# gleb-kov/wordpiece

Measured on AMD Instinct MI355X. Metric: input MB/s tokenized (bert-base-cased vocab; offline stand-in: synthetic BERT-like vocab), higher is better.
Workload: dtype int32

## Files before the change

### include/wordpiece_amd.h

```cpp
#ifndef WORDPIECE_AMD_H
#define WORDPIECE_AMD_H

#include <stddef.h>
#include <stdint.h>

#ifdef __cplusplus
extern "C" {
#endif

#define WP_OK 0
#define WP_ERR_EMPTY_WORD 1
#define WP_ERR_TOO_LARGE 2
#define WP_ERR_HIP 3
#define WP_ERR_NO_DEVICE 4
#define WP_ERR_IO 5
#define WP_ERR_ARG 6

typedef struct wp_vocab wp_vocab;

int wp_vocab_create(const char *const *lines, const size_t *line_bytes, size_t n_lines,
                    wp_vocab **out);
int wp_vocab_create_packed(const char *buf, const int64_t *offsets, int64_t n_lines,
                           wp_vocab **out);
int wp_vocab_from_file(const char *vocab_file, wp_vocab **out);
// ... 33 lines not shown
typedef struct { int32_t max_len, cls_id, sep_id, pad_id, pairs, truncation, stride, unit; } wp_inputs_spec;
typedef struct { int32_t *input_ids, *token_type_ids, *lengths, *sample; uint32_t *offsets; } wp_inputs;
int wp_linear_encode_inputs(wp_vocab *v, const char *utf8, size_t nbytes, const int64_t *doc_off, size_t n_docs,
                            const wp_inputs_spec *spec, wp_inputs *out, size_t *n_out, size_t *n_samples);
int wp_linear_encode_inputs_device(wp_vocab *v, const void *d_utf8, size_t nbytes, const int64_t *d_doc_off, size_t n_docs,
                                   const wp_inputs_spec *spec, const wp_inputs *d_out, size_t capacity_rows,
                                   size_t *n_out, size_t *n_samples);

typedef struct { int32_t max_len, cls_id, sep_id, pad_id, mask_id, ignore_id, whole_word, reserved;
                 uint64_t select_q32, mask_q32, random_q32, seed, row_base; } wp_mask_spec;
int wp_word_ids(wp_vocab *v, const int32_t *input_ids, const int32_t *lengths, size_t n_rows, const wp_mask_spec *spec,
                int32_t **word_ids);
int wp_word_ids_device(wp_vocab *v, const int32_t *d_input_ids, const int32_t *d_lengths, size_t n_rows,
                       const wp_mask_spec *spec, int32_t *d_word_ids);
int wp_mlm_mask(wp_vocab *v, const int32_t *input_ids, const int32_t *lengths, size_t n_rows, const wp_mask_spec *spec,
                int32_t **masked, int32_t **labels, int32_t **word_ids);
int wp_mlm_mask_device(wp_vocab *v, const int32_t *d_input_ids, const int32_t *d_lengths, size_t n_rows,
                       const wp_mask_spec *spec, int32_t *d_masked, int32_t *d_labels, int32_t *d_word_ids);
typedef struct {
  int64_t n_rows;
  int64_t n_words;
  int64_t n_selected;
  int64_t n_selected_units;
  int64_t n_masked, n_random, n_kept;
  int32_t whole_word, reserved;
} wp_mask_stats;
int wp_get_mask_stats(const wp_vocab *v, wp_mask_stats *out);

typedef struct { int32_t max_len, cleanup, terminator, n_skip; int32_t skip_ids[8]; } wp_detok_spec;
int wp_detokenize(wp_vocab *v, const int32_t *ids, const int64_t *row_splits, const int32_t *lengths, size_t n_rows,
                  const wp_detok_spec *spec, char **text, int64_t **text_off, size_t *n_bytes);
int wp_detokenize_device(wp_vocab *v, const int32_t *d_ids, const int64_t *d_row_splits, const int32_t *d_lengths,
                         size_t n_rows, const wp_detok_spec *spec, const void **d_text, const int64_t **d_text_off,
                         size_t *n_bytes);
int64_t wp_detok_piece(const wp_vocab *v, int64_t id, int form, int cleanup, char *buf, size_t cap);
typedef struct { int64_t n_rows, n_cells, n_kept, n_skipped, n_dropped, n_bytes; } wp_detok_stats;
int wp_get_detok_stats(const wp_vocab *v, wp_detok_stats *out);

int wp_linear_encode_multi(wp_vocab *v, const char *utf8, size_t nbytes, const int *devices,
                           int n_devices, int32_t **ids, size_t *n_ids);

int wp_linear_encode_batch(wp_vocab *v, const char *const *texts, const size_t *nbytes, size_t n_texts,
                           int32_t **ids, size_t *n_ids);

typedef int (*wp_text_source)(void *user, size_t index, const char **utf8, size_t *nbytes);
typedef void (*wp_ids_sink)(void *user, size_t index, const int32_t *ids, size_t n_ids);
int wp_linear_encode_stream(wp_vocab *v, wp_text_source next, wp_ids_sink out, void *user);

int wp_reserve(wp_vocab *v, size_t nbytes);

int wp_trim(wp_vocab *v);

int wp_linear_encode_file(const char *text_file, const char *vocab_file, int32_t **ids,
                          size_t *n_ids);
int wp_linear_encode_external(const char *text_file, const char *vocab_file, const char *out_file,
                              size_t memory_limit);

int wp_fast_encode(wp_vocab *v, const char *utf8, size_t nbytes, int32_t **ids, size_t *n_ids);
int wp_fast_encode_device(wp_vocab *v, const void *d_utf8, size_t nbytes, const int32_t **d_ids,
                          size_t *n_ids);
int wp_fast_encode_file(const char *text_file, const char *vocab_file, int32_t **ids, size_t *n_ids);
int wp_fast_encode_external(const char *text_file, const char *vocab_file, const char *out_file,
                            size_t memory_limit);
int64_t wp_vocab_token_utf8(const wp_vocab *v, int64_t i, char *buf, size_t cap);

#define WP_OPT_FULL_DEPTH 1
#define WP_OPT_DEVICE 2
#define WP_OPT_KEEP_DEBUG 3
#define WP_OPT_STAGE_TIMING 4
#define WP_OPT_LCP_KASAI 5
#define WP_OPT_COVER_ANCHORS 7
#define WP_OPT_ARENA_GUARD 8
#define WP_OPT_DEVICES 9
#define WP_OPT_VOCAB_IN_S 10
#define WP_OPT_SPARSE_EMIT 11
#define WP_OPT_INDEXED_ROUND0 12
#define WP_OPT_SORT_BLANKS 13
#define WP_OPT_NORMALIZE 14
#define WP_NORM_CLEAN 1
#define WP_NORM_LOWER 2
#define WP_NORM_STRIP_ACCENTS 4
#define WP_NORM_BERT_UNCASED 7
#define WP_OPT_LATE_REFINE 15
int wp_set_option(wp_vocab *v, int option, int64_t value);

int wp_normalize_cp(int flags, uint32_t cp, uint32_t out[3]);
int wp_normalize_device(wp_vocab *v, const void *d_utf8, size_t nbytes, int flags, const void **d_out, size_t *out_bytes);
int wp_normalize(wp_vocab *v, const char *utf8, size_t nbytes, int flags, char **out, size_t *out_bytes);

typedef struct {
  int64_t n_bytes, n_text, n_total, alphabet, longest_token, n_ids;
  int32_t symbol_bits, symbols_per_key, rounds, sorted_depth, full_depth;
  int64_t radix_pass_elems;
  int32_t radix_passes;
  int64_t active_per_round[40];
  double ms_total, ms_decode, ms_sa, ms_lcp, ms_scan, ms_walk;
  double ms_radix_scatter;
  int64_t n_anchors;
  int32_t anchor_mode;
  double ms_h2d, ms_d2h;
  int64_t radix_digit_bytes;
  double ms_host_total;
  int32_t guard_zones;
  int32_t n_devices;
  int32_t vocab_in_s;
  int32_t reserved0;
  int64_t needed_after_round0;
  int32_t key_bits;
  int32_t staged_emit;
  int32_t rank_in_pass;
  int32_t trie_refine;
  int64_t arena_bytes;
  int32_t list_retries;
  int32_t hist_in_keys;
  int64_t radix_pass_bytes;
  int64_t round0_candidates;
  int32_t round0_keys_only;
  int32_t offsets_unit;
  int64_t round0_sorted;
  int64_t n_rows, rows_truncated;
  int32_t rows_route;
} wp_stats;
int wp_get_stats(const wp_vocab *v, wp_stats *out);
typedef struct {
  int32_t normalize;
  int64_t norm_bytes;
  double ms_normalize;
} wp_norm_stats;
int wp_get_norm_stats(const wp_vocab *v, wp_norm_stats *out);
typedef struct {
  int64_t n_wide_words;
  int64_t n_long_words;
  int32_t lean;
  int32_t max_anchor_gap;
} wp_walk_stats;
int wp_get_walk_stats(const wp_vocab *v, wp_walk_stats *out);
typedef struct {
  int64_t n_groups;
  int64_t n_entries;
  int64_t n_large_groups;
  int64_t n_large_entries;
  int64_t trie_nodes;
  int32_t sort_bits;
  int32_t key_lookup;
  int32_t symbol_bytes;
  int32_t reserved;
} wp_refine_stats;
int wp_get_refine_stats(const wp_vocab *v, wp_refine_stats *out);
typedef struct {
  int32_t early;
  int32_t reserved;
  double ms_sort_to_scan;
} wp_refine_sched;
int wp_get_refine_sched(const wp_vocab *v, wp_refine_sched *out);
typedef struct {
  int64_t n_samples, n_out;
  int64_t n_cut;
  int64_t n_windowed;
  int32_t pairs, truncation, stride, reserved;
} wp_inputs_stats;
int wp_get_inputs_stats(const wp_vocab *v, wp_inputs_stats *out);

int wp_linear_debug_fetch(const wp_vocab *v, int which, int32_t *out, size_t capacity,
                          size_t *n_out);

void wp_free(void *p);
const char *wp_last_error(void);
int wp_device_count(void);

#ifdef __cplusplus
}
#endif
#endif
```

### wordpiece_amd/__init__.py

```python
import ctypes as C
import os
import weakref

import numpy as np

_HERE = os.path.dirname(os.path.abspath(__file__))
LIB_PATH = os.environ.get("WP_LIB") or os.path.join(_HERE, "libwordpiece_amd.so")

WP_OPT_FULL_DEPTH, WP_OPT_DEVICE, WP_OPT_KEEP_DEBUG, WP_OPT_STAGE_TIMING, WP_OPT_LCP_KASAI = 1, 2, 3, 4, 5
WP_OPT_COVER_ANCHORS, WP_OPT_ARENA_GUARD, WP_OPT_DEVICES, WP_OPT_VOCAB_IN_S = 7, 8, 9, 10
WP_OPT_SPARSE_EMIT = 11
WP_OPT_INDEXED_ROUND0 = 12
WP_OPT_SORT_BLANKS = 13
WP_OPT_NORMALIZE = 14
WP_OPT_LATE_REFINE = 15
WP_NORM_CLEAN, WP_NORM_LOWER, WP_NORM_STRIP_ACCENTS, WP_NORM_BERT_UNCASED = 1, 2, 4, 7
WP_OFFSETS_BYTES, WP_OFFSETS_CODE_POINTS = 0, 1
_OFFSET_UNITS = {"byte": WP_OFFSETS_BYTES, "char": WP_OFFSETS_CODE_POINTS}
WP_TRUNC_LONGEST_FIRST, WP_TRUNC_ONLY_FIRST, WP_TRUNC_ONLY_SECOND = 0, 1, 2
_TRUNCATIONS = {"longest_first": WP_TRUNC_LONGEST_FIRST, "only_first": WP_TRUNC_ONLY_FIRST,
                "only_second": WP_TRUNC_ONLY_SECOND}

ABI_SYMBOLS = [
    "wp_vocab_create", "wp_vocab_create_packed", "wp_vocab_from_file", "wp_vocab_destroy", "wp_vocab_size",
    "wp_vocab_unk_id", "wp_vocab_token_flags", "wp_vocab_token_len", "wp_linear_encode",
    "wp_linear_encode_device", "wp_linear_encode_file", "wp_linear_encode_external", "wp_set_option",
    "wp_get_stats", "wp_linear_debug_fetch", "wp_free", "wp_last_error", "wp_device_count",
    "wp_linear_encode_multi", "wp_reserve", "wp_fast_encode", "wp_fast_encode_device", "wp_fast_encode_file",
    "wp_fast_encode_external", "wp_vocab_token_utf8", "wp_trim", "wp_linear_encode_batch", "wp_linear_encode_stream",
    "wp_linear_encode_offsets", "wp_linear_encode_offsets_device",
    "wp_linear_encode_rows", "wp_linear_encode_rows_device", "wp_linear_encode_padded", "wp_linear_encode_padded_device",
    "wp_normalize_cp", "wp_normalize_device", "wp_normalize", "wp_get_norm_stats", "wp_get_walk_stats",
    "wp_get_refine_stats", "wp_get_refine_sched",
    "wp_linear_encode_inputs", "wp_linear_encode_inputs_device", "wp_get_inputs_stats",
    "wp_word_ids", "wp_word_ids_device", "wp_mlm_mask", "wp_mlm_mask_device", "wp_get_mask_stats",
    "wp_detokenize", "wp_detokenize_device", "wp_detok_piece", "wp_get_detok_stats",
]


class WordPieceError(RuntimeError):
    """Mirrors the std::runtime_error the reference throws (message = wp_last_error())."""


class Stats(C.Structure):
    _fields_ = [("n_bytes", C.c_int64), ("n_text", C.c_int64), ("n_total", C.c_int64), ("alphabet", C.c_int64),
                ("longest_token", C.c_int64), ("n_ids", C.c_int64),
                ("symbol_bits", C.c_int32), ("symbols_per_key", C.c_int32), ("rounds", C.c_int32),
                ("sorted_depth", C.c_int32), ("full_depth", C.c_int32),
                ("radix_pass_elems", C.c_int64), ("radix_passes", C.c_int32),
                ("active_per_round", C.c_int64 * 40),
                ("ms_total", C.c_double), ("ms_decode", C.c_double), ("ms_sa", C.c_double), ("ms_lcp", C.c_double),
                ("ms_scan", C.c_double), ("ms_walk", C.c_double), ("ms_radix_scatter", C.c_double),
                ("n_anchors", C.c_int64), ("anchor_mode", C.c_int32), ("ms_h2d", C.c_double), ("ms_d2h", C.c_double),
                ("radix_digit_bytes", C.c_int64), ("ms_host_total", C.c_double), ("guard_zones", C.c_int32),
                ("n_devices", C.c_int32), ("vocab_in_s", C.c_int32), ("reserved0", C.c_int32),
                ("needed_after_round0", C.c_int64), ("key_bits", C.c_int32), ("staged_emit", C.c_int32),
                ("rank_in_pass", C.c_int32), ("trie_refine", C.c_int32), ("arena_bytes", C.c_int64),
                ("list_retries", C.c_int32), ("hist_in_keys", C.c_int32), ("radix_pass_bytes", C.c_int64),
                ("round0_candidates", C.c_int64), ("round0_keys_only", C.c_int32), ("offsets_unit", C.c_int32),
                ("round0_sorted", C.c_int64), ("n_rows", C.c_int64), ("rows_truncated", C.c_int64),
                ("rows_route", C.c_int32)]

    def as_dict(self):
        d = {k: getattr(self, k) for k, _ in self._fields_ if k != "active_per_round"}
        d["active_per_round"] = [int(x) for x in self.active_per_round[:max(self.rounds, 0)]]
        return d


class NormStats(C.Structure):
    _fields_ = [("normalize", C.c_int32), ("norm_bytes", C.c_int64), ("ms_normalize", C.c_double)]


class WalkStats(C.Structure):
    _fields_ = [("n_wide_words", C.c_int64), ("n_long_words", C.c_int64), ("lean", C.c_int32),
                ("max_anchor_gap", C.c_int32)]


class RefineStats(C.Structure):
    _fields_ = [("n_groups", C.c_int64), ("n_entries", C.c_int64), ("n_large_groups", C.c_int64),
                ("n_large_entries", C.c_int64), ("trie_nodes", C.c_int64), ("sort_bits", C.c_int32),
                ("key_lookup", C.c_int32), ("symbol_bytes", C.c_int32), ("reserved", C.c_int32)]


class RefineSched(C.Structure):
    _fields_ = [("early", C.c_int32), ("reserved", C.c_int32), ("ms_sort_to_scan", C.c_double)]


class InputsSpec(C.Structure):
    _fields_ = [("max_len", C.c_int32), ("cls_id", C.c_int32), ("sep_id", C.c_int32), ("pad_id", C.c_int32),
                ("pairs", C.c_int32), ("truncation", C.c_int32), ("stride", C.c_int32), ("unit", C.c_int32)]


class Inputs(C.Structure):
    _fields_ = [("input_ids", C.c_void_p), ("token_type_ids", C.c_void_p), ("lengths", C.c_void_p), ("sample", C.c_void_p),
                ("offsets", C.c_void_p)]


class InputsStats(C.Structure):
    _fields_ = [("n_samples", C.c_int64), ("n_out", C.c_int64), ("n_cut", C.c_int64), ("n_windowed", C.c_int64),
                ("pairs", C.c_int32), ("truncation", C.c_int32), ("stride", C.c_int32), ("reserved", C.c_int32)]


class MaskSpec(C.Structure):
    _fields_ = [("max_len", C.c_int32), ("cls_id", C.c_int32), ("sep_id", C.c_int32), ("pad_id", C.c_int32),
                ("mask_id", C.c_int32), ("ignore_id", C.c_int32), ("whole_word", C.c_int32), ("reserved", C.c_int32),
                ("select_q32", C.c_uint64), ("mask_q32", C.c_uint64), ("random_q32", C.c_uint64), ("seed", C.c_uint64),
                ("row_base", C.c_uint64)]


class MaskStats(C.Structure):
    _fields_ = [("n_rows", C.c_int64), ("n_words", C.c_int64), ("n_selected", C.c_int64), ("n_selected_units", C.c_int64),
                ("n_masked", C.c_int64), ("n_random", C.c_int64), ("n_kept", C.c_int64), ("whole_word", C.c_int32),
                ("reserved", C.c_int32)]


class DetokSpec(C.Structure):
    _fields_ = [("max_len", C.c_int32), ("cleanup", C.c_int32), ("terminator", C.c_int32), ("n_skip", C.c_int32),
                ("skip_ids", C.c_int32 * 8)]


class DetokStats(C.Structure):
    _fields_ = [("n_rows", C.c_int64), ("n_cells", C.c_int64), ("n_kept", C.c_int64), ("n_skipped", C.c_int64),
                ("n_dropped", C.c_int64), ("n_bytes", C.c_int64)]


_TEXT_SOURCE = C.CFUNCTYPE(C.c_int, C.c_void_p, C.c_size_t, C.POINTER(C.c_void_p), C.POINTER(C.c_size_t))
_IDS_SINK = C.CFUNCTYPE(None, C.c_void_p, C.c_size_t, C.POINTER(C.c_int32), C.c_size_t)

_lib = None


def lib():
    global _lib
    if _lib is None:
        if not os.path.exists(LIB_PATH):
            raise WordPieceError("HIP extension missing: %s (run `python -m wordpiece_amd.build`)" % LIB_PATH)
        L = C.CDLL(LIB_PATH)
        vp, i32p = C.c_void_p, C.POINTER(C.c_int32)
        L.wp_vocab_create.argtypes = [C.POINTER(C.c_char_p), C.POINTER(C.c_size_t), C.c_size_t, C.POINTER(vp)]
        L.wp_vocab_create_packed.argtypes = [C.c_char_p, C.POINTER(C.c_int64), C.c_int64, C.POINTER(vp)]
        L.wp_vocab_from_file.argtypes = [C.c_char_p, C.POINTER(vp)]
        L.wp_vocab_destroy.argtypes = [vp]
        L.wp_vocab_destroy.restype = None
        L.wp_vocab_size.argtypes = [vp]
        L.wp_vocab_size.restype = C.c_int64
        L.wp_vocab_unk_id.argtypes = [vp]
        L.wp_vocab_unk_id.restype = C.c_int32
        L.wp_vocab_token_flags.argtypes = [vp, C.c_int64]
        L.wp_vocab_token_flags.restype = C.c_int32
        L.wp_vocab_token_len.argtypes = [vp, C.c_int64]
        L.wp_vocab_token_len.restype = C.c_int64
        L.wp_linear_encode.argtypes = [vp, C.c_char_p, C.c_size_t, C.POINTER(i32p), C.POINTER(C.c_size_t)]
        L.wp_linear_encode_device.argtypes = [vp, vp, C.c_size_t, C.POINTER(vp), C.POINTER(C.c_size_t)]
        u32p = C.POINTER(C.c_uint32)
        L.wp_linear_encode_offsets.argtypes = [vp, C.c_char_p, C.c_size_t, C.c_int, C.POINTER(i32p), C.POINTER(u32p),
                                               C.POINTER(C.c_size_t)]
        L.wp_linear_encode_offsets_device.argtypes = [vp, vp, C.c_size_t, C.c_int, C.POINTER(vp), C.POINTER(vp),
                                                      C.POINTER(C.c_size_t)]
        i64p = C.POINTER(C.c_int64)
        L.wp_linear_encode_rows.argtypes = [vp, C.c_char_p, C.c_size_t, i64p, C.c_size_t, C.c_int, C.POINTER(i32p),
                                            C.POINTER(i64p), C.POINTER(u32p), C.POINTER(C.c_size_t), C.POINTER(C.c_size_t)]
        L.wp_linear_encode_rows_device.argtypes = [vp, vp, C.c_size_t, vp, C.c_size_t, C.c_int, C.POINTER(vp), C.POINTER(vp),
                                                   C.POINTER(vp), C.POINTER(C.c_size_t), C.POINTER(C.c_size_t)]
        L.wp_linear_encode_padded.argtypes = [vp, C.c_char_p, C.c_size_t, i64p, C.c_size_t, C.c_int, C.c_int32, C.c_int32,
                                              C.c_int32, C.POINTER(i32p), C.POINTER(i32p), C.POINTER(C.c_size_t)]
        L.wp_linear_encode_padded_device.argtypes = [vp, vp, C.c_size_t, vp, C.c_size_t, C.c_int, C.c_int32, C.c_int32,
                                                     C.c_int32, vp, vp, C.c_size_t, C.POINTER(C.c_size_t)]
        L.wp_linear_encode_inputs.argtypes = [vp, C.c_char_p, C.c_size_t, i64p, C.c_size_t, C.POINTER(InputsSpec),
                                              C.POINTER(Inputs), C.POINTER(C.c_size_t), C.POINTER(C.c_size_t)]
        L.wp_linear_encode_inputs_device.argtypes = [vp, vp, C.c_size_t, vp, C.c_size_t, C.POINTER(InputsSpec),
                                                     C.POINTER(Inputs), C.c_size_t, C.POINTER(C.c_size_t),
                                                     C.POINTER(C.c_size_t)]
        L.wp_get_inputs_stats.argtypes = [vp, C.POINTER(InputsStats)]
        L.wp_word_ids.argtypes = [vp, i32p, i32p, C.c_size_t, C.POINTER(MaskSpec), C.POINTER(i32p)]
        L.wp_word_ids_device.argtypes = [vp, vp, vp, C.c_size_t, C.POINTER(MaskSpec), vp]
        L.wp_mlm_mask.argtypes = [vp, i32p, i32p, C.c_size_t, C.POINTER(MaskSpec), C.POINTER(i32p), C.POINTER(i32p),
                                  C.POINTER(i32p)]
        L.wp_mlm_mask_device.argtypes = [vp, vp, vp, C.c_size_t, C.POINTER(MaskSpec), vp, vp, vp]
        L.wp_get_mask_stats.argtypes = [vp, C.POINTER(MaskStats)]
        L.wp_detokenize.argtypes = [vp, i32p, C.POINTER(C.c_int64), i32p, C.c_size_t, C.POINTER(DetokSpec),
                                    C.POINTER(C.c_void_p), C.POINTER(C.POINTER(C.c_int64)), C.POINTER(C.c_size_t)]
        L.wp_detokenize_device.argtypes = [vp, vp, vp, vp, C.c_size_t, C.POINTER(DetokSpec), C.POINTER(C.c_void_p),
                                           C.POINTER(C.c_void_p), C.POINTER(C.c_size_t)]
        L.wp_detok_piece.argtypes = [vp, C.c_int64, C.c_int, C.c_int, C.c_char_p, C.c_size_t]
        L.wp_detok_piece.restype = C.c_int64
        L.wp_get_detok_stats.argtypes = [vp, C.POINTER(DetokStats)]
        L.wp_linear_encode_multi.argtypes = [vp, C.c_char_p, C.c_size_t, C.POINTER(C.c_int), C.c_int, C.POINTER(i32p),
                                             C.POINTER(C.c_size_t)]
        L.wp_reserve.argtypes = [vp, C.c_size_t]
        L.wp_linear_encode_stream.argtypes = [vp, _TEXT_SOURCE, _IDS_SINK, vp]
        L.wp_linear_encode_batch.argtypes = [vp, C.POINTER(C.c_char_p), C.POINTER(C.c_size_t), C.c_size_t, C.POINTER(i32p),
                                             C.POINTER(C.c_size_t)]
        L.wp_trim.argtypes = [vp]
        L.wp_fast_encode.argtypes = [vp, C.c_char_p, C.c_size_t, C.POINTER(i32p), C.POINTER(C.c_size_t)]
        L.wp_fast_encode_device.argtypes = [vp, vp, C.c_size_t, C.POINTER(vp), C.POINTER(C.c_size_t)]
        L.wp_fast_encode_file.argtypes = [C.c_char_p, C.c_char_p, C.POINTER(i32p), C.POINTER(C.c_size_t)]
        L.wp_fast_encode_external.argtypes = [C.c_char_p, C.c_char_p, C.c_char_p, C.c_size_t]
        L.wp_vocab_token_utf8.argtypes = [vp, C.c_int64, C.c_char_p, C.c_size_t]
        L.wp_vocab_token_utf8.restype = C.c_int64
        L.wp_linear_encode_file.argtypes = [C.c_char_p, C.c_char_p, C.POINTER(i32p), C.POINTER(C.c_size_t)]
        L.wp_linear_encode_external.argtypes = [C.c_char_p, C.c_char_p, C.c_char_p, C.c_size_t]
        L.wp_normalize_cp.argtypes = [C.c_int, C.c_uint32, C.POINTER(C.c_uint32)]
        L.wp_normalize_device.argtypes = [vp, vp, C.c_size_t, C.c_int, C.POINTER(vp), C.POINTER(C.c_size_t)]
        L.wp_normalize.argtypes = [vp, C.c_char_p, C.c_size_t, C.c_int, C.POINTER(vp), C.POINTER(C.c_size_t)]
        L.wp_set_option.argtypes = [vp, C.c_int, C.c_int64]
        L.wp_get_stats.argtypes = [vp, C.POINTER(Stats)]
        L.wp_get_norm_stats.argtypes = [vp, C.POINTER(NormStats)]
        L.wp_get_walk_stats.argtypes = [vp, C.POINTER(WalkStats)]
        L.wp_get_refine_stats.argtypes = [vp, C.POINTER(RefineStats)]
        if hasattr(L, "wp_get_refine_sched"):
            L.wp_get_refine_sched.argtypes = [vp, C.POINTER(RefineSched)]
        L.wp_linear_debug_fetch.argtypes = [vp, C.c_int, i32p, C.c_size_t, C.POINTER(C.c_size_t)]
        L.wp_free.argtypes = [vp]
        L.wp_free.restype = None
        L.wp_last_error.restype = C.c_char_p
        L.wp_device_count.restype = C.c_int
        _lib = L
    return _lib


def _check(rc):
    if rc != 0:
        raise WordPieceError(lib().wp_last_error().decode("utf8", "replace"))


def _bytes(x):
    return bytes(x) if isinstance(x, (bytes, bytearray, memoryview)) else x.encode("utf8")


class Vocab:

    def __init__(self, lines=None, file=None, device=None, normalize=0):
        self._h = C.c_void_p()
        if file is not None:
            _check(lib().wp_vocab_from_file(_bytes(file), C.byref(self._h)))
        else:
            ls = [_bytes(w) for w in lines]
            off = np.zeros(len(ls) + 1, dtype=np.int64)
            if ls:
                off[1:] = np.cumsum([len(w) for w in ls])
            _check(lib().wp_vocab_create_packed(b"".join(ls), off.ctypes.data_as(C.POINTER(C.c_int64)), len(ls),
                                                C.byref(self._h)))
        self._device = None if device is None else int(device)
        if device is not None:
            self.set_option(WP_OPT_DEVICE, device)
        if normalize:
            self.set_option(WP_OPT_NORMALIZE, normalize)
        self._normalize = int(normalize)

    def __del__(self):
        if getattr(self, "_h", None) and _lib is not None:
            _lib.wp_vocab_destroy(self._h)
            self._h = None

    def __len__(self):
        return lib().wp_vocab_size(self._h)

    @property
    def unk_id(self):
        return lib().wp_vocab_unk_id(self._h)

    def token_flags(self, i):
        return lib().wp_vocab_token_flags(self._h, i)

    def token_len(self, i):
        return lib().wp_vocab_token_len(self._h, i)

    def set_option(self, opt, value):
        _check(lib().wp_set_option(self._h, opt, int(value)))
        if opt == WP_OPT_NORMALIZE:
            self._normalize = int(value)
        if opt == WP_OPT_DEVICE:
            self._device = int(value)

    def normalize(self, text, flags=None):
        b = _bytes(text)
        out = C.c_void_p()
        n = C.c_size_t()
        _check(lib().wp_normalize(self._h, b, len(b), self._normalize if flags is None else int(flags), C.byref(out), C.byref(n)))
        if n.value == 0:
            return b""
        try:
            return C.string_at(out, n.value)
        finally:
            lib().wp_free(out)

    def normalize_tensor(self, text, flags=None, copy=True):
        import torch
        if text.dtype != torch.uint8 or not text.is_cuda or not text.is_contiguous():
            raise WordPieceError("normalize_tensor needs a contiguous uint8 CUDA/HIP tensor")
        nbytes = text.numel()
        if text.data_ptr() % 4 != 0 or nbytes % 4 != 0:
            padded = torch.zeros((nbytes + 19) // 16 * 16, dtype=torch.uint8, device=text.device)
            padded[:nbytes] = text
            text = padded
        torch.cuda.current_stream(text.device).synchronize()
        d_out = C.c_void_p()
        n = C.c_size_t()
        _check(lib().wp_normalize_device(self._h, C.c_void_p(text.data_ptr()), nbytes,
                                         self._normalize if flags is None else int(flags), C.byref(d_out), C.byref(n)))
        if n.value == 0:
            return torch.zeros(0, dtype=torch.uint8, device=text.device)
        view = torch.as_tensor(DeviceIds(d_out.value, n.value, typestr="|u1"), device=text.device)
        return view.clone() if copy else view

    def stats(self):
        s = Stats()
        _check(lib().wp_get_stats(self._h, C.byref(s)))
        d = s.as_dict()
        ns = NormStats()
        _check(lib().wp_get_norm_stats(self._h, C.byref(ns)))
        d.update({k: getattr(ns, k) for k, _ in ns._fields_})
        return d

    def walk_stats(self):
        ws = WalkStats()
        _check(lib().wp_get_walk_stats(self._h, C.byref(ws)))
        return {k: int(getattr(ws, k)) for k, _ in ws._fields_}

    def refine_stats(self):
        rs = RefineStats()
        _check(lib().wp_get_refine_stats(self._h, C.byref(rs)))
        return {k: int(getattr(rs, k)) for k, _ in rs._fields_ if k != "reserved"}

    def refine_sched(self):
        rs = RefineSched()
        _check(lib().wp_get_refine_sched(self._h, C.byref(rs)))
        return {"early": int(rs.early), "ms_sort_to_scan": float(rs.ms_sort_to_scan)}

    def encode(self, text):
        b = _bytes(text)
        ids = C.POINTER(C.c_int32)()
        n = C.c_size_t()
        _check(lib().wp_linear_encode(self._h, b, len(b), C.byref(ids), C.byref(n)))
        return _adopt_ids(ids, n.value)

    def encode_with_offsets(self, text, unit="byte"):
        b = _bytes(text)
        ids = C.POINTER(C.c_int32)()
        offs = C.POINTER(C.c_uint32)()
        n = C.c_size_t()
        _check(lib().wp_linear_encode_offsets(self._h, b, len(b), _offset_unit(unit), C.byref(ids), C.byref(offs),
                                              C.byref(n)))
        if n.value == 0:
            return np.zeros(0, dtype=np.int32), np.zeros((0, 2), dtype=np.uint32)
        return _adopt_ids(ids, n.value), _adopt_block(offs, (n.value, 2))

    def encode_device_with_offsets(self, d_ptr, nbytes, unit="byte"):
        d_ids = C.c_void_p()
        d_offs = C.c_void_p()
        n = C.c_size_t()
        _check(lib().wp_linear_encode_offsets_device(self._h, C.c_void_p(d_ptr), nbytes, _offset_unit(unit), C.byref(d_ids),
                                                     C.byref(d_offs), C.byref(n)))
        return d_ids.value, d_offs.value, n.value

    def encode_rows(self, docs=None, text=None, doc_offsets=None, offsets=None):
        b, off = _docs_arg(docs, text, doc_offsets)
        unit = -1 if offsets is None else _offset_unit(offsets)
        ids, splits, offs = C.POINTER(C.c_int32)(), C.POINTER(C.c_int64)(), C.POINTER(C.c_uint32)()
        n, rows = C.c_size_t(), C.c_size_t()
        _check(lib().wp_linear_encode_rows(self._h, b, len(b), _i64_ptr(off), 0 if off is None else len(off) - 1, unit,
                                           C.byref(ids), C.byref(splits), C.byref(offs), C.byref(n), C.byref(rows)))
        out = (_adopt_ids(ids, n.value), _adopt_block(splits, (rows.value + 1,)))
        if offsets is None:
            return out
        return out + (_adopt_block(offs, (n.value, 2)) if n.value else np.zeros((0, 2), dtype=np.uint32),)

    def encode_padded(self, docs=None, text=None, doc_offsets=None, max_len=128, cls_id=None, sep_id=None, pad_id=0):
        b, off = _docs_arg(docs, text, doc_offsets)
        ids, lens = C.POINTER(C.c_int32)(), C.POINTER(C.c_int32)()
        rows = C.c_size_t()
        _check(lib().wp_linear_encode_padded(self._h, b, len(b), _i64_ptr(off), 0 if off is None else len(off) - 1,
                                             int(max_len), _special(cls_id), _special(sep_id), int(pad_id), C.byref(ids),
                                             C.byref(lens), C.byref(rows)))
        if rows.value == 0:
            return np.zeros((0, int(max_len)), dtype=np.int32), np.zeros(0, dtype=np.int32)
        return _adopt_block(ids, (rows.value, int(max_len))), _adopt_block(lens, (rows.value,))

    def _rows_tensor_args(self, text, doc_offsets):
        import torch
        if text.dtype != torch.uint8 or not text.is_cuda or not text.is_contiguous():
            raise WordPieceError("a documents call on tensors needs a contiguous uint8 CUDA/HIP text tensor")
        nbytes = text.numel()
        if text.data_ptr() % 4 != 0 or nbytes % 4 != 0:
            padded = torch.zeros((nbytes + 19) // 16 * 16, dtype=torch.uint8, device=text.device)
            padded[:nbytes] = text
            text = padded
        if doc_offsets is not None:
            if doc_offsets.dtype != torch.int64 or doc_offsets.device != text.device or doc_offsets.dim() != 1 or \
                    doc_offsets.numel() < 1:
                raise WordPieceError("doc_offsets must be a 1-d int64 tensor on the text's device")
            doc_offsets = doc_offsets.contiguous()
        torch.cuda.current_stream(text.device).synchronize()
        return text, nbytes, doc_offsets

    def encode_rows_tensor(self, text, doc_offsets=None, offsets=None, copy=True):
        import torch
        text, nbytes, doc_offsets = self._rows_tensor_args(text, doc_offsets)
        unit = -1 if offsets is None else _offset_unit(offsets)
        d_ids, d_splits, d_offs = C.c_void_p(), C.c_void_p(), C.c_void_p()
        n, rows = C.c_size_t(), C.c_size_t()
        _check(lib().wp_linear_encode_rows_device(
            self._h, C.c_void_p(text.data_ptr()), nbytes, None if doc_offsets is None else C.c_void_p(doc_offsets.data_ptr()),
            0 if doc_offsets is None else doc_offsets.numel() - 1, unit, C.byref(d_ids), C.byref(d_splits), C.byref(d_offs),
            C.byref(n), C.byref(rows)))
        dev = text.device
        ids = torch.as_tensor(DeviceIds(d_ids.value, n.value), device=dev) if n.value else \
            torch.zeros(0, dtype=torch.int32, device=dev)
        splits = torch.as_tensor(DeviceIds(d_splits.value, rows.value + 1, typestr="<i8"), device=dev)
        out = (ids, splits)
        if offsets is not None:
# ... 579 lines not shown
```

### wordpiece_amd/csrc/context.h

```cpp
#pragma once
#include <array>
#include <cstring>
#include <memory>
#include <mutex>
#include <string>
#include <vector>

#include "../../include/wordpiece_amd.h"
#include "code.h"
#include "decode.h"
#include "detok.h"
#include "radix_sort.h"
#include "scanline.h"
#include "suffix_array.h"
#include "vocab.h"

namespace wp {

static thread_local std::string g_last_error;

struct EnvOptions {
  bool arena_guard;
  bool vocab_in_s;
  bool sparse_emit;
  bool no_pool;
  static bool flag(const char *name) {
    const char *e = getenv(name);
    return e && atoi(e) != 0;
  }
  static const EnvOptions &get() {
    static const EnvOptions o{flag("WP_ARENA_GUARD"), flag("WP_VOCAB_IN_S"), flag("WP_SPARSE_EMIT"), flag("WP_NO_CONTEXT_POOL")};
    return o;
  }
};

struct DeviceBuffer {
  void *p = nullptr;
  size_t cap = 0;
  void ensure(size_t bytes, bool slack = true) {
    if (bytes <= cap) return;
    if (p) WP_HIP(hipFree(p));
    p = nullptr;
    cap = 0;
    size_t want = slack ? bytes + bytes / 16 + (1 << 20) : bytes;
    WP_HIP(hipMalloc(&p, want));
    cap = want;
  }
  void release() {
    if (p) (void)hipFree(p);
    p = nullptr;
    cap = 0;
  }
};

static size_t text_room(size_t len) { return len + 64; }
static void zero_text_tail(void *d_text, size_t len, hipStream_t st) {
  WP_HIP(hipMemsetAsync(static_cast<char *>(d_text) + (len & ~static_cast<size_t>(15)), 0, 32, st));
}

constexpr size_t kGuardBytes = 256;
constexpr uint32_t kGuardWord = 0xA5C3F00Du;

__global__ __launch_bounds__(kBlock) void guard_fill_kernel(char *base, const unsigned long long *offs, int count) {
  const int z = blockIdx.x;
  if (z >= count) return;
  uint32_t *g = reinterpret_cast<uint32_t *>(base + offs[z]);
  if (threadIdx.x < kGuardBytes / 4) g[threadIdx.x] = kGuardWord;
}
__global__ __launch_bounds__(kBlock) void guard_check_kernel(const char *base, const unsigned long long *offs, int count,
                                                             uint32_t *bad) {
  const int z = blockIdx.x;
  if (z >= count) return;
  const uint32_t *g = reinterpret_cast<const uint32_t *>(base + offs[z]);
  const bool broken = threadIdx.x < kGuardBytes / 4 && g[threadIdx.x] != kGuardWord;
  if (__syncthreads_or(broken) && threadIdx.x == 0) {
    atomicAdd(&bad[0], 1u);
    atomicMin(&bad[1], static_cast<uint32_t>(z) + 1u);
  }
}

struct Arena {
  DeviceBuffer *buf;
  size_t off = 0, planned = 0;
  bool planning = true, guard = false;
  std::vector<unsigned long long> zones;
  explicit Arena(DeviceBuffer *b, bool g = false) : buf(b), guard(g) {}
  template <typename T>
  T *take(size_t count) {
    size_t bytes = (count * sizeof(T) + 255) & ~static_cast<size_t>(255);
    size_t o = off;
    off += bytes;
    if (guard) {
      if (!planning) zones.push_back(off);
      off += kGuardBytes;
    }
    if (planning) return nullptr;
    if (off > planned) throw std::logic_error("arena: the allocation sequence differs from the planned one");
    return reinterpret_cast<T *>(static_cast<char *>(buf->p) + o);
  }
  void commit() {
    buf->ensure(off + (guard ? 8 * 512 : 0));
    planned = off;
    off = 0;
    planning = false;
  }
  unsigned long long *zone_table() const {
    return reinterpret_cast<unsigned long long *>(static_cast<char *>(buf->p) + ((off + 255) & ~static_cast<size_t>(255)));
  }
  void arm(hipStream_t st) {
    if (!guard || zones.empty()) return;
    if (zones.size() > 500) throw std::logic_error("arena guard: too many allocations");
    WP_HIP(hipMemcpyAsync(zone_table(), zones.data(), zones.size() * sizeof(unsigned long long), hipMemcpyHostToDevice, st));
    WP_HIP(hipStreamSynchronize(st));
    hipLaunchKernelGGL(guard_fill_kernel, dim3(zones.size()), dim3(kBlock), 0, st, static_cast<char *>(buf->p), zone_table(),
                       static_cast<int>(zones.size()));
  }
  void check(hipStream_t st, uint32_t *bad) const {
    if (!guard || zones.empty()) return;
    hipLaunchKernelGGL(guard_check_kernel, dim3(zones.size()), dim3(kBlock), 0, st, static_cast<const char *>(buf->p),
                       zone_table(), static_cast<int>(zones.size()), bad);
  }
};

static int bit_length(uint64_t v) {
  int b = 0;
  while (v) {
    b++;
    v >>= 1;
  }
  return b;
}

constexpr int kScalars = 56;
constexpr int kScalarCps = 0;
constexpr int kScalarAlphabet = 1;
constexpr int kScalarInvalid = 2;
constexpr int kScalarList = 4;
constexpr int kScalarListEntries = kScalarList + 0;
constexpr int kScalarListGroups = kScalarList + 1;
constexpr int kScalarListLargeGroups = kScalarList + 2;
constexpr int kScalarListLargeEntries = kScalarList + 3;
constexpr int kScalarListWanted = 8;
constexpr int kScalarIds = 9;
constexpr int kScalarAnchors = 10;
constexpr int kScalarAnchorGap = 11;
constexpr int kScalarLongWords = 12;
constexpr int kScalarWideWords = 13;
constexpr int kScalarCps64 = 14;
constexpr int kScalarGuard = 16;
constexpr int kScalarGuardBad = kScalarGuard + 0;
constexpr int kScalarGuardFirst = kScalarGuard + 1;
constexpr int kScalarSplitTotals = 18;
constexpr int kScalarAlphaWord0 = 20;
constexpr int kScalarRows = 21, kScalarRowsBad = 22, kScalarRowsCut = 23;
constexpr int kScalarCand = 24;
constexpr int kScalarKept = 25;
constexpr int kScalarSrcRows = 26;
constexpr int kScalarInCut = 27, kScalarInRows = 28, kScalarInWindowed = 30;
constexpr int kScalarFree31 = 31;
constexpr int kScalarMask = 32;
constexpr int kScalarDetokLast = 44, kScalarDetokBad = 46;
constexpr int kScalarFree47 = 47;
constexpr int kScalarDetok = 48;
constexpr int kScalarNormBytes = kScalarCps;
constexpr int kScalarNormCps = kScalarAlphabet;
constexpr int kScalarNormSrcCps = kScalarListEntries;
constexpr int kScalarNormBytes64 = kScalarCps64;

struct ScalarRange {
  int first, words;
};
constexpr ScalarRange kScalarLayout[] = {
    {kScalarCps, 1},         {kScalarAlphabet, 1},   {kScalarInvalid, 2},         {kScalarListEntries, 1},
    {kScalarListGroups, 1},  {kScalarListLargeGroups, 1}, {kScalarListLargeEntries, 1}, {kScalarListWanted, 1},
    {kScalarIds, 1},         {kScalarAnchors, 1},    {kScalarAnchorGap, 1},       {kScalarLongWords, 1},
    {kScalarWideWords, 1},   {kScalarCps64, 2},      {kScalarGuardBad, 1},        {kScalarGuardFirst, 1},
    {kScalarSplitTotals, 2},      {kScalarAlphaWord0, 1}, {kScalarRows, 1},            {kScalarRowsBad, 1},
    {kScalarRowsCut, 1},     {kScalarCand, 1},       {kScalarKept, 1},            {kScalarSrcRows, 1},
    {kScalarInCut, 1},       {kScalarInRows, 2},     {kScalarInWindowed, 1},      {kScalarFree31, 1},
    {kScalarMask, 12},       {kScalarDetokLast, 2},  {kScalarDetokBad, 1},        {kScalarFree47, 1},
    {kScalarDetok, 8}};
constexpr int scalar_end(int slot) {
  for (const ScalarRange &r : kScalarLayout) {
    if (slot < r.first + r.words) return r.first + r.words;
  }
  return kScalars;
}
constexpr bool scalar_layout_ok() {
  int at = 0;
  for (const ScalarRange &r : kScalarLayout) {
    if (r.first != at || r.words < 1 || (r.words % 2 == 0 && r.first % 2 != 0)) return false;
    at += r.words;
  }
  return at == kScalars;
}
static_assert(scalar_layout_ok(), "the scalar table must cover d_scalars word by word, 64-bit slots on even words");
static_assert(kScalarList % 2 == 0 && kScalarListLargeGroups % 2 == 0, "both halves of the list block are also read as 64-bit words");

struct RowsCall {
  const long long *d_doc_off = nullptr;
  size_t n_docs = 0;
  int unit = -1;
  size_t capacity = SIZE_MAX;
  size_t n_rows = 0;
  const long long *d_starts = nullptr;
  const long long *d_row_splits = nullptr;
  uint32_t *d_line_cnt = nullptr;
};

enum SideEvent { kEvFork, kEvJoin, kEvScalars, kEvKeysFree, kEvPartition, kEvTrieNodes, kEvLargeSorted, kEvKeysBuilt, kEvCandCount,
                 kEvSpine, kEvKept, kEvSorted, kEvListBuilt, kEvRoundDone, kSideEvents };
enum TimingMark { kMarkStart, kMarkCounted, kMarkSymbols, kMarkSorted, kMarkLcp, kMarkScanned, kMarkWalked, kMarkNormStart,
                  kMarkRound0, kTimingMarks, kMarkNormEnd = kMarkStart };

struct Context {
  int device = 0;
  hipStream_t stream = nullptr;
  hipStream_t stream2 = nullptr;
  hipStream_t stream3 = nullptr;
  hipEvent_t evs[kSideEvents] = {};
  uint32_t *d_stream = nullptr, *d_elig_start = nullptr, *d_elig_info = nullptr, *d_soft = nullptr;
  uint32_t *d_vocab_word_idx = nullptr, *d_vocab_word_bits = nullptr;
  uint8_t *d_cls_bmp = nullptr;
  uint32_t *d_lt_chain_len = nullptr, *d_lt_chain_off = nullptr, *d_lt_child_begin = nullptr, *d_lt_child_cp = nullptr,
           *d_lt_child_node = nullptr, *d_elig_node = nullptr, *d_elig_subtree = nullptr;
  int32_t *d_elig_id = nullptr, *d_tok_len = nullptr;
  uint8_t *d_tok_class = nullptr;
  DetokRec *d_detok_rec = nullptr;
  uint8_t *d_detok_pool = nullptr;
  size_t detok_pool_bytes = 0;
  unsigned long long *d_trie_key = nullptr;
  uint32_t *d_trie_child = nullptr;
  int32_t *d_trie_id = nullptr;
  DeviceBuffer text_buf, a_buf, b_buf, fmt_buf;
  DeviceBuffer text_buf2, ids_stage[2];
  DeviceBuffer rows_in, rows_out, pad_buf;
  DeviceBuffer inputs_buf;
  DeviceBuffer detok_in, detok_aux, detok_out;
  uint16_t *d_norm_index = nullptr;
  uint32_t *d_norm_pages = nullptr, *d_norm_pool = nullptr;
  DeviceBuffer norm_buf, norm_aux, norm_map;
  hipStream_t up_stream = nullptr, down_stream = nullptr;
  hipEvent_t pipe_ev[4] = {};
  uint32_t *d_used = nullptr, *d_lut = nullptr, *d_scan_tmp = nullptr;
  uint32_t *d_scalars = nullptr;
  uint8_t *d_code = nullptr;
  size_t list_hint = 0;
  SymbolCode code_cache;
  bool code_cached = false;
  uint32_t code_alphabet = 0;
  int code_bits = 0, code_lo = 0, code_uses = 0;
  double code_blank_share = 0.0;
  uint8_t *h_code = nullptr;
  uint32_t *d_symhist = nullptr;
  uint32_t *h_scalars = nullptr;
  RadixStats rstats;
  hipEvent_t ev[kTimingMarks] = {};
  const int32_t *d_ids = nullptr;
  const uint32_t *d_offs = nullptr;
  struct {
    const void *sym = nullptr;
    int sym_bytes = 0;
    const uint32_t *sa = nullptr, *cps = nullptr;
    const RankEntry *rank = nullptr;
    const int32_t *lcp = nullptr;
    const uint8_t *cls = nullptr;
    StepTable steps{};
    int32_t *best_scratch = nullptr;
    size_t n = 0, n_text = 0;
  } dbg;
  std::array<DeviceBuffer *, 17> buffers() {
    return {&text_buf, &a_buf,    &b_buf,   &fmt_buf,    &text_buf2, &ids_stage[0], &ids_stage[1], &rows_in,   &rows_out,
            &pad_buf,  &inputs_buf, &norm_buf, &norm_aux, &norm_map, &detok_in,     &detok_aux,    &detok_out};
  }
  Context() = default;
  Context(const Context &) = delete;
  Context &operator=(const Context &) = delete;
  ~Context();
};

struct DeviceGuard {
  int prev = -1;
  DeviceGuard() {
    if (hipGetDevice(&prev) != hipSuccess) prev = -1;
  }
  ~DeviceGuard() {
    if (prev >= 0) (void)hipSetDevice(prev);
  }
  DeviceGuard(const DeviceGuard &) = delete;
  DeviceGuard &operator=(const DeviceGuard &) = delete;
};

#ifdef WP_DEBUG_BOUNDS
static void take_oob(int first, int count, unsigned int *oob) {
  WP_HIP(hipMemcpyFromSymbol(oob, HIP_SYMBOL(g_wp_oob), count * sizeof(unsigned int), first * sizeof(unsigned int)));
  bool any = false;
  for (int i = 0; i < count; i++) any = any || oob[i] != 0;
  if (!any) return;
  const unsigned int zero[kBoundSites] = {};
  WP_HIP(hipMemcpyToSymbol(HIP_SYMBOL(g_wp_oob), zero, count * sizeof(unsigned int), first * sizeof(unsigned int)));
}
#endif

}

using namespace wp;

struct EncodeStats : wp_stats {
  int32_t normalize;
  int64_t norm_bytes;
  double ms_normalize;
  wp_walk_stats walk;
  wp_refine_stats refine;
  wp_refine_sched sched;
  wp_inputs_stats inputs;
  int32_t inputs_call;
  wp_mask_stats mask;
  int32_t mask_call;
  wp_detok_stats detok;
  int32_t detok_call;
};

#ifndef WP_LATE_REFINE_DEFAULT
#define WP_LATE_REFINE_DEFAULT 0
#endif

struct wp_vocab {
  HostVocab hv;
  std::unique_ptr<Context> ctx;
  std::vector<std::unique_ptr<Context>> multi;
  int device = -1;
  bool full_depth = false, keep_debug = false, stage_timing = false, lcp_kasai = false, cover_anchors = false;
  bool arena_guard = false;
  bool sparse_emit = false;
  bool vocab_in_s = false;
  bool indexed_round0 = false;
  bool sort_blanks = false;
  bool late_refine = WP_LATE_REFINE_DEFAULT != 0;
  int normalize = 0;
  int n_devices = 1;
  EncodeStats stats{};
  ~wp_vocab();
};

namespace wp {

template <typename... T>
static void free_dev(T *&...p) {
  (((p ? (void)hipFree(p) : (void)0), p = nullptr), ...);
}

static void free_vocab_tables(Context *c) {
  free_dev(c->d_stream, c->d_elig_start, c->d_elig_info, c->d_soft, c->d_elig_id, c->d_tok_len, c->d_tok_class, c->d_detok_rec, c->d_detok_pool, c->d_trie_key,
           c->d_trie_child, c->d_trie_id, c->d_vocab_word_idx, c->d_vocab_word_bits, c->d_cls_bmp, c->d_lt_chain_len,
           c->d_lt_chain_off, c->d_lt_child_begin, c->d_lt_child_cp, c->d_lt_child_node, c->d_elig_node, c->d_elig_subtree);
}

template <size_t N>
static void destroy_events(hipEvent_t (&events)[N]) {
  for (auto &e : events) {
    if (e) (void)hipEventDestroy(e);
    e = nullptr;
  }
}

static void destroy_context(Context *c) {
  if (!c) return;
  bool owns = c->stream || c->stream2 || c->stream3 || c->d_used || c->d_lut || c->d_scan_tmp || c->d_scalars || c->d_code ||
              c->d_symhist || c->h_scalars || c->h_code || c->d_stream;
  for (DeviceBuffer *b : c->buffers()) owns = owns || b->p;
  if (!owns) return;
  DeviceGuard keep;
  (void)hipSetDevice(c->device);
  free_vocab_tables(c);
  free_dev(c->d_used, c->d_lut, c->d_scan_tmp, c->d_scalars, c->d_code, c->d_symhist, c->d_norm_index, c->d_norm_pages, c->d_norm_pool);
  if (c->h_scalars) (void)hipHostFree(c->h_scalars);
  if (c->h_code) (void)hipHostFree(c->h_code);
  c->h_scalars = nullptr;
  c->h_code = nullptr;
  for (DeviceBuffer *b : c->buffers()) b->release();
  destroy_events(c->pipe_ev);
  destroy_events(c->ev);
  destroy_events(c->evs);
  for (hipStream_t *s : {&c->up_stream, &c->down_stream, &c->stream3, &c->stream2, &c->stream}) {
    if (*s) (void)hipStreamDestroy(*s);
    *s = nullptr;
  }
}
Context::~Context() { destroy_context(this); }

template <typename T>
static T *upload(const std::vector<T> &v, hipStream_t st) {
  T *d = nullptr;
  WP_HIP(hipMalloc(&d, std::max<size_t>(v.size(), 1) * sizeof(T)));
  if (!v.empty()) WP_HIP(hipMemcpyAsync(d, v.data(), v.size() * sizeof(T), hipMemcpyHostToDevice, st));
  return d;
}

static constexpr size_t kPoolArenaBytes = size_t(256) << 20;
static constexpr size_t kPoolContexts = 4;
static std::mutex g_pool_mu;
static std::vector<std::unique_ptr<Context>> &context_pool() {
  static auto *pool = new std::vector<std::unique_ptr<Context>>();
  return *pool;
}

static void release_arenas(Context *c) {
  for (DeviceBuffer *b : c->buffers()) b->release();
  c->d_ids = nullptr;
  c->d_offs = nullptr;
  c->dbg = {};
}

static void park_context(std::unique_ptr<Context> c) {
  if (!c) return;
  const bool no_pool = EnvOptions::get().no_pool;
  DeviceGuard keep;
  (void)hipSetDevice(c->device);
  if (!no_pool && hipStreamSynchronize(c->stream) == hipSuccess && hipStreamSynchronize(c->stream2) == hipSuccess &&
      hipStreamSynchronize(c->stream3) == hipSuccess) {
    free_vocab_tables(c.get());
// ... 4 lines not shown
    c->d_offs = nullptr;
    c->dbg = {};
    std::lock_guard<std::mutex> g(g_pool_mu);
    if (context_pool().size() < kPoolContexts) {
      context_pool().push_back(std::move(c));
      return;
    }
  }
  destroy_context(c.get());
}

static void upload_vocab_tables(Context *c, const HostVocab &hv) {
  c->d_stream = upload(hv.stream, c->stream);
  c->d_elig_start = upload(hv.elig_start, c->stream);
  c->d_elig_info = upload(hv.elig_info, c->stream);
  c->d_elig_id = upload(hv.elig_id, c->stream);
  c->d_tok_len = upload(hv.tok_len, c->stream);
  c->d_soft = upload(hv.soft, c->stream);
  c->d_vocab_word_idx = upload(hv.used_word_idx, c->stream);
  c->d_vocab_word_bits = upload(hv.used_word_bits, c->stream);
  c->d_cls_bmp = upload(hv.cls_bmp, c->stream);
  c->d_lt_chain_len = upload(hv.lt_chain_len, c->stream);
  c->d_lt_chain_off = upload(hv.lt_chain_off, c->stream);
  c->d_lt_child_begin = upload(hv.lt_child_begin, c->stream);
  c->d_lt_child_cp = upload(hv.lt_child_cp, c->stream);
  c->d_lt_child_node = upload(hv.lt_child_node, c->stream);
  c->d_elig_node = upload(hv.elig_node, c->stream);
  c->d_elig_subtree = upload(hv.elig_subtree, c->stream);
  {
    std::vector<unsigned long long> tk(hv.trie_key.begin(), hv.trie_key.end());
    c->d_trie_key = upload(tk, c->stream);
    WP_HIP(hipStreamSynchronize(c->stream));
  }
  c->d_trie_child = upload(hv.trie_child, c->stream);
  c->d_trie_id = upload(hv.trie_id, c->stream);
  WP_HIP(hipStreamSynchronize(c->stream));
}

static int device_count_or_throw() {
  int count = 0;
  if (hipGetDeviceCount(&count) != hipSuccess || count == 0) {
    throw HipError("no HIP device available: the Linear WordPiece path has no CPU fallback");
  }
  return count;
}

static std::unique_ptr<Context> make_context(const wp_vocab *v, int device) {
  const int count = device_count_or_throw();
  if (device >= 0) {
    if (device >= count) throw std::invalid_argument("no such HIP device: " + std::to_string(device));
  } else {
    WP_HIP(hipGetDevice(&device));
  }
  WP_HIP(hipSetDevice(device));
  std::unique_ptr<Context> c;
  {
    std::lock_guard<std::mutex> g(g_pool_mu);
    auto &pool = context_pool();
    for (size_t i = 0; i < pool.size(); i++) {
      if (pool[i]->device == device) {
        c = std::move(pool[i]);
        pool.erase(pool.begin() + static_cast<long>(i));
        break;
      }
    }
  }
  if (c) {
    upload_vocab_tables(c.get(), v->hv);
    return c;
  }
  c.reset(new Context());
  c->device = device;
  WP_HIP(hipStreamCreateWithFlags(&c->stream, hipStreamNonBlocking));
  WP_HIP(hipStreamCreateWithFlags(&c->stream2, hipStreamNonBlocking));
  WP_HIP(hipStreamCreateWithFlags(&c->stream3, hipStreamNonBlocking));
  for (auto &e : c->evs) WP_HIP(hipEventCreateWithFlags(&e, hipEventDisableTiming));
  WP_HIP(hipMalloc(&c->d_used, sizeof(uint32_t) * kCpWords));
  WP_HIP(hipMalloc(&c->d_lut, sizeof(uint32_t) * kCpTableSize));
  WP_HIP(hipMalloc(&c->d_scan_tmp, sizeof(uint32_t) * kCpWords));
  WP_HIP(hipMalloc(&c->d_scalars, sizeof(uint32_t) * kScalars));
  WP_HIP(hipMalloc(&c->d_code, 512 + 256 + kDecodeTableBytes));
  WP_HIP(hipHostMalloc(&c->h_code, 512 + 256 + kDecodeTableBytes));
  WP_HIP(hipMalloc(&c->d_symhist, sizeof(uint32_t) * 256));
  WP_HIP(hipHostMalloc(&c->h_scalars, sizeof(uint32_t) * kScalars));
  for (auto &e : c->ev) WP_HIP(hipEventCreate(&e));
  upload_vocab_tables(c.get(), v->hv);
  return c;
}

static Context *get_context(wp_vocab *v) {
  if (!v->ctx) v->ctx = make_context(v, v->device);
  WP_HIP(hipSetDevice(v->ctx->device));
  return v->ctx.get();
}

static void queue_scalars(Context *c, int last, hipStream_t st) {
  WP_HIP(hipMemcpyAsync(c->h_scalars, c->d_scalars, sizeof(uint32_t) * scalar_end(last), hipMemcpyDeviceToHost, st));
}
static void fetch_scalars(Context *c, int last) {
  queue_scalars(c, last, c->stream);
  WP_HIP(hipStreamSynchronize(c->stream));
}
static void clear_scalars(Context *c, int first, int last, hipStream_t st) {
  WP_HIP(hipMemsetAsync(c->d_scalars + first, 0, sizeof(uint32_t) * (scalar_end(last) - first), st));
}

}
```

### wordpiece_amd/csrc/encoder.hip

```cpp
#include <fcntl.h>
#include <sys/mman.h>
#include <sys/stat.h>
#include <unistd.h>

#include <atomic>
#include <chrono>
#include <cstring>
#include <fstream>
#include <functional>
#include <future>
#include <memory>
#include <mutex>
#include <thread>
#include <unordered_map>
#include <vector>

#include "../../include/wordpiece_amd.h"
#include "context.h"
#include "detok.h"
#include "fast_path.h"
#include "format.h"
#include "inputs.h"
#include "linear_path.h"
#include "mask.h"
// ... 52 lines not shown
  try {
  std::unique_ptr<wp_vocab> v(new wp_vocab());
  if (const char *e = getenv("WP_DEVICES")) {
    v->n_devices = std::strcmp(e, "all") == 0 ? -1 : std::max(1, atoi(e));
  }
  std::string err = v->hv.build(lines);
  if (!err.empty()) {
    g_last_error = err;
    return WP_ERR_EMPTY_WORD;
  }
  *out = v.release();
  return WP_OK;
  } catch (const std::exception &e) {
    g_last_error = e.what();
    return WP_ERR_ARG;
  } catch (...) {
    g_last_error = "unknown exception while building the vocabulary";
    return WP_ERR_ARG;
  }
}

extern "C" {

int wp_vocab_create(const char *const *lines, const size_t *line_bytes, size_t n_lines, wp_vocab **out) {
  std::vector<std::pair<const char *, size_t>> ls;
  ls.reserve(n_lines);
  for (size_t i = 0; i < n_lines; i++) ls.emplace_back(lines[i], line_bytes[i]);
  return vocab_from_lines(ls, out);
}

int wp_vocab_create_packed(const char *buf, const int64_t *offsets, int64_t n_lines, wp_vocab **out) {
  std::vector<std::pair<const char *, size_t>> ls;
  ls.reserve(static_cast<size_t>(n_lines));
  for (int64_t i = 0; i < n_lines; i++) ls.emplace_back(buf + offsets[i], static_cast<size_t>(offsets[i + 1] - offsets[i]));
  return vocab_from_lines(ls, out);
}

int wp_vocab_from_file(const char *vocab_file, wp_vocab **out) {
  std::ifstream fin(vocab_file);
  std::vector<std::string> words;
  std::string w;
  while (std::getline(fin, w)) words.push_back(w);
  std::vector<std::pair<const char *, size_t>> ls;
  for (auto &s : words) ls.emplace_back(s.data(), s.size());
  return vocab_from_lines(ls, out);
}

void wp_vocab_destroy(wp_vocab *v) {
  if (!v) return;
  try {
    delete v;
  } catch (...) {
  }
}
int64_t wp_vocab_size(const wp_vocab *v) { return static_cast<int64_t>(v->hv.tokens.size()); }
int32_t wp_vocab_unk_id(const wp_vocab *v) { return v->hv.unk_id; }
int32_t wp_vocab_token_flags(const wp_vocab *v, int64_t i) {
  return token_flags(v->hv.tokens[static_cast<size_t>(i)]);
}
int64_t wp_vocab_token_len(const wp_vocab *v, int64_t i) {
  return static_cast<int64_t>(v->hv.tokens[static_cast<size_t>(i)].word.size());
}

int wp_set_option(wp_vocab *v, int option, int64_t value) {
  switch (option) {
    case WP_OPT_FULL_DEPTH: v->full_depth = value != 0; return WP_OK;
    case WP_OPT_DEVICE:
      if (v->ctx) {
        g_last_error = "device already bound";
        return WP_ERR_ARG;
      }
      v->device = static_cast<int>(value);
      return WP_OK;
    case WP_OPT_KEEP_DEBUG: v->keep_debug = value != 0; return WP_OK;
    case WP_OPT_STAGE_TIMING: v->stage_timing = value != 0; return WP_OK;
    case WP_OPT_LCP_KASAI: v->lcp_kasai = value != 0; return WP_OK;
    case WP_OPT_COVER_ANCHORS: v->cover_anchors = value != 0; return WP_OK;
    case WP_OPT_ARENA_GUARD: v->arena_guard = value != 0; return WP_OK;
    case WP_OPT_VOCAB_IN_S: v->vocab_in_s = value != 0; return WP_OK;
    case WP_OPT_SPARSE_EMIT: v->sparse_emit = value != 0; return WP_OK;
    case WP_OPT_INDEXED_ROUND0: v->indexed_round0 = value != 0; return WP_OK;
    case WP_OPT_SORT_BLANKS: v->sort_blanks = value != 0; return WP_OK;
    case WP_OPT_LATE_REFINE: v->late_refine = value != 0; return WP_OK;
    case WP_OPT_NORMALIZE:
      if (!known_norm_flags(value)) {
        g_last_error = "WP_OPT_NORMALIZE: unknown flag bits (WP_NORM_CLEAN | WP_NORM_LOWER | WP_NORM_STRIP_ACCENTS)";
        return WP_ERR_ARG;
      }
      v->normalize = static_cast<int>(value);
      return WP_OK;
    case WP_OPT_DEVICES: v->n_devices = value < 0 ? -1 : static_cast<int>(std::max<int64_t>(value, 1)); return WP_OK;
  }
  g_last_error = "unknown option";
  return WP_ERR_ARG;
}

int wp_normalize_cp(int flags, uint32_t cp, uint32_t out[3]) {
  if (!known_norm_flags(flags) || cp >= 0x110000u || (cp >= 0xd800u && cp < 0xe000u)) return -1;
  uint32_t o[3] = {0, 0, 0};
  const int n = norm_cp(host_norm_tables(), flags, cp, o);
  for (int i = 0; i < n; i++) out[i] = o[i];
  return n;
}

int wp_normalize_device(wp_vocab *v, const void *d_utf8, size_t nbytes, int flags, const void **d_out, size_t *out_bytes) {
  return guarded([&] {
    *d_out = nullptr;
    *out_bytes = 0;
    if (!known_norm_flags(flags)) throw std::invalid_argument("normalize: unknown flag bits");
    if (nbytes == 0) return;
    check_device_text(d_utf8);
    Context *c = get_context(v);
    NormResult r;
    normalize_on_device(c, static_cast<const uint8_t *>(d_utf8), nbytes, flags, false, false, r);
    WP_HIP(hipStreamSynchronize(c->stream));
    *d_out = r.nbytes ? r.text : nullptr;
    *out_bytes = r.nbytes;
  });
}

int wp_get_stats(const wp_vocab *v, wp_stats *out) {
  *out = v->stats;
  return WP_OK;
}

int wp_get_norm_stats(const wp_vocab *v, wp_norm_stats *out) {
  out->normalize = v->stats.normalize;
  out->norm_bytes = v->stats.norm_bytes;
  out->ms_normalize = v->stats.ms_normalize;
  return WP_OK;
}

int wp_get_walk_stats(const wp_vocab *v, wp_walk_stats *out) {
  *out = v->stats.walk;
  return WP_OK;
}

int wp_get_refine_stats(const wp_vocab *v, wp_refine_stats *out) {
  *out = v->stats.refine;
  return WP_OK;
}

int wp_get_refine_sched(const wp_vocab *v, wp_refine_sched *out) {
  if (!v || !out) {
    g_last_error = "wp_get_refine_sched: NULL handle or out pointer";
    return WP_ERR_ARG;
  }
  *out = v->stats.sched;
  return WP_OK;
}

int wp_get_inputs_stats(const wp_vocab *v, wp_inputs_stats *out) {
  *out = v->stats.inputs;
  if (!v->stats.inputs_call) out->n_out = -1;
  return WP_OK;
}

int wp_linear_encode_device(wp_vocab *v, const void *d_utf8, size_t nbytes, const int32_t **d_ids, size_t *n_ids) {
  return guarded([&] {
    check_device_text(d_utf8);
    size_t n = 0;
    Context *c = get_context(v);
    encode_on_device(v, c, static_cast<const uint8_t *>(d_utf8), nbytes, &n, v->stats);
    v->stats.n_devices = 1;
    *d_ids = n ? c->d_ids : nullptr;
    *n_ids = n;
  });
}

}

namespace {
struct PinnedPool {
  std::mutex mu;
  std::unordered_map<void *, size_t> owned;
  std::vector<std::pair<size_t, void *>> pooled;
  static constexpr size_t kMaxPooledBlocks = 4;
  static constexpr size_t kMaxPooledBytes = size_t(6) << 30;
  void *take(size_t bytes) {
    {
      std::lock_guard<std::mutex> g(mu);
      size_t best = pooled.size();
      for (size_t i = 0; i < pooled.size(); i++) {
        if (pooled[i].first >= bytes && (best == pooled.size() || pooled[i].first < pooled[best].first)) best = i;
      }
      if (best != pooled.size()) {
        void *p = pooled[best].second;
        pooled.erase(pooled.begin() + static_cast<long>(best));
        return p;
      }
    }
    void *p = nullptr;
    const size_t want = bytes + bytes / 8 + 4096;
    WP_HIP(hipHostMalloc(&p, want));
    std::lock_guard<std::mutex> g(mu);
    owned[p] = want;
    return p;
  }
  bool give_back(void *p) {
    size_t cap = 0;
    {
      std::lock_guard<std::mutex> g(mu);
      auto it = owned.find(p);
      if (it == owned.end()) return false;
      cap = it->second;
      size_t bytes = cap;
      for (auto &b : pooled) bytes += b.first;
      if (pooled.size() < kMaxPooledBlocks && bytes <= kMaxPooledBytes) {
        pooled.emplace_back(cap, p);
        return true;
      }
      owned.erase(it);
    }
    (void)hipHostFree(p);
    return true;
  }
  void trim() {
    std::vector<std::pair<size_t, void *>> drop;
    {
      std::lock_guard<std::mutex> g(mu);
      drop.swap(pooled);
      for (auto &b : drop) owned.erase(b.second);
    }
    for (auto &b : drop) (void)hipHostFree(b.second);
  }
};
PinnedPool &id_pool() {
  static PinnedPool *pool = new PinnedPool();
  return *pool;
}
struct PinnedBlock {
// ... 1347 lines not shown
  DeviceBuffer *tb[2] = {&c->text_buf, &c->text_buf2};
  const int device = c->device;
  std::atomic<long long> up_us{0};
  auto upload = [&](const char *text, size_t len, int slot) -> std::string {
    try {
      if (len == 0) return "";
      const auto t_up = wp_clock::now();
      WP_HIP(hipSetDevice(device));
      upload_text(*tb[slot], c->up_stream, text, len);
      WP_HIP(hipStreamSynchronize(c->up_stream));
      up_us += static_cast<long long>(ms_since(t_up) * 1e3);
      return "";
    } catch (const std::exception &e) {
      return e.what()[0] ? e.what() : "upload failed";
    }
  };
  EncodeStats total{};
  const char *cur_text = nullptr, *next_text = nullptr;
  size_t cur_len = 0, next_len = 0;
  bool have = next(0, &cur_text, &cur_len);
  if (have) {
    tb[0]->ensure(text_room(cur_len));
    const std::string err = upload(cur_text, cur_len, 0);
    if (!err.empty()) throw HipError(err);
  }
  std::unique_ptr<PinnedBlock> in_flight;
  size_t in_flight_n = 0, in_flight_i = 0;
  int in_flight_slot = 0;
  for (size_t i = 0; have; i++) {
    const int slot = static_cast<int>(i & 1);
    const bool more = next(i + 1, &next_text, &next_len);
    std::future<std::string> next_up;
    if (more) {
      tb[slot ^ 1]->ensure(text_room(next_len));
      next_up = std::async(std::launch::async, upload, next_text, next_len, slot ^ 1);
    }
    struct Wait {
      std::future<std::string> &f;
      ~Wait() {
        if (f.valid()) f.wait();
      }
    } wait_up{next_up};
    size_t n = 0;
    EncodeStats st{};
    if (cur_len) encode_on_device(v, c, static_cast<const uint8_t *>(tb[slot]->p), cur_len, &n, st);
    std::unique_ptr<PinnedBlock> blk(new PinnedBlock(std::max<size_t>(n, 1) * sizeof(int32_t)));
    if (n) {
      c->ids_stage[slot].ensure(n * sizeof(int32_t));
      WP_HIP(hipMemcpyAsync(c->ids_stage[slot].p, c->d_ids, n * sizeof(int32_t), hipMemcpyDeviceToDevice, c->stream));
      WP_HIP(hipEventRecord(c->pipe_ev[slot], c->stream));
      WP_HIP(hipStreamWaitEvent(c->down_stream, c->pipe_ev[slot], 0));
      WP_HIP(hipMemcpyAsync(blk->p, c->ids_stage[slot].p, n * sizeof(int32_t), hipMemcpyDeviceToHost, c->down_stream));
      WP_HIP(hipEventRecord(c->pipe_ev[2 + slot], c->down_stream));
    }
    if (in_flight) {
      if (in_flight_n) WP_HIP(hipEventSynchronize(c->pipe_ev[2 + in_flight_slot]));
      deliver(in_flight_i, *in_flight, in_flight_n);
    }
    in_flight = std::move(blk);
    in_flight_n = n;
    in_flight_i = i;
    in_flight_slot = slot;
    total.n_bytes += st.n_bytes;
    total.n_text += st.n_text;
    total.n_total += st.n_total;
    total.n_ids += st.n_ids;
    total.ms_total += st.ms_total;
    total.normalize = std::max(total.normalize, st.normalize);
    total.norm_bytes += st.norm_bytes;
    total.ms_normalize += st.ms_normalize;
    total.walk.n_wide_words += st.walk.n_wide_words;
    total.walk.n_long_words += st.walk.n_long_words;
    total.walk.max_anchor_gap = std::max(total.walk.max_anchor_gap, st.walk.max_anchor_gap);
    if (i == 0) total.walk.lean = st.walk.lean;
    {
      const wp_refine_stats sum = total.refine;
      if (i == 0) total.refine = st.refine;
      total.refine.n_groups = sum.n_groups + st.refine.n_groups;
      total.refine.n_entries = sum.n_entries + st.refine.n_entries;
      total.refine.n_large_groups = sum.n_large_groups + st.refine.n_large_groups;
      total.refine.n_large_entries = sum.n_large_entries + st.refine.n_large_entries;
    }
    if (i == 0) total.sched = st.sched;
    total.rounds = std::max(total.rounds, st.rounds);
    if (next_up.valid()) {
      const std::string err = next_up.get();
      if (!err.empty()) throw HipError(err);
    }
    have = more;
    cur_text = next_text;
    cur_len = next_len;
  }
  if (in_flight) {
    if (in_flight_n) WP_HIP(hipEventSynchronize(c->pipe_ev[2 + in_flight_slot]));
    deliver(in_flight_i, *in_flight, in_flight_n);
  }
  v->stats = total;
  v->stats.n_devices = 1;
  v->stats.ms_h2d = static_cast<double>(up_us.load()) / 1e3;
  v->stats.ms_host_total = ms_since(t_all);
}
}

extern "C" {

int wp_linear_encode_batch(wp_vocab *v, const char *const *texts, const size_t *nbytes, size_t n_texts, int32_t **ids,
                           size_t *n_ids) {
  return guarded([&] {
    for (size_t i = 0; i < n_texts; i++) {
      ids[i] = nullptr;
      n_ids[i] = 0;
    }
    std::vector<void *> got(n_texts, nullptr);
    try {
      encode_pipeline(
          v,
          [&](size_t i, const char **t, size_t *len) {
            if (i >= n_texts) return false;
            *t = texts[i];
            *len = nbytes[i];
            return true;
          },
          [&](size_t i, PinnedBlock &blk, size_t n) {
            n_ids[i] = n;
            if (n) got[i] = blk.release();
          });
    } catch (...) {
      for (void *p : got) {
        if (p) id_pool().give_back(p);
      }
      for (size_t i = 0; i < n_texts; i++) n_ids[i] = 0;
      throw;
    }
    for (size_t i = 0; i < n_texts; i++) ids[i] = static_cast<int32_t *>(got[i]);
  });
}

int wp_linear_encode_stream(wp_vocab *v, wp_text_source next, wp_ids_sink out, void *user) {
  return guarded([&] {
    if (!next || !out) throw std::invalid_argument("wp_linear_encode_stream: null callback");
    encode_pipeline(
        v, [&](size_t i, const char **t, size_t *len) { return next(user, i, t, len) != 0; },
        [&](size_t i, PinnedBlock &blk, size_t n) { out(user, i, n ? static_cast<const int32_t *>(blk.p) : nullptr, n); });
  });
}

int wp_trim(wp_vocab *v) {
  return guarded([&] {
    auto drop = [](Context *c) {
      if (!c) return;
      WP_HIP(hipSetDevice(c->device));
      WP_HIP(hipStreamSynchronize(c->stream));
      WP_HIP(hipStreamSynchronize(c->stream2));
      release_arenas(c);
    };
    if (v) {
      drop(v->ctx.get());
      for (auto &c : v->multi) drop(c.get());
    }
    {
      std::lock_guard<std::mutex> g(g_pool_mu);
      for (auto &c : context_pool()) drop(c.get());
    }
    id_pool().trim();
  });
}
// ... 294 lines not shown
```

### wordpiece_amd/csrc/linear_path.h

```cpp
#pragma once
#include <functional>

#include "context.h"
#include "local_sort.h"
#include "prune.h"
#include "trie.h"
#include "offsets.h"
#include "normalize.h"
#include "rows.h"
#include "walk.h"

namespace wp {

struct ListOverflow {
  size_t wanted;
};

__global__ void needed_list_clamp_kernel(uint32_t *__restrict__ totals, uint32_t cap, uint32_t *__restrict__ wanted) {
  if (totals[0] > cap) {
    *wanted = totals[0];
    totals[0] = 0;
    totals[1] = 0;
  }
}

constexpr double kBlankDropMinShare = 1.0 / 16;

#ifdef WP_DEBUG_BOUNDS
__device__ unsigned int g_wp_sorted_sig[6];
__global__ __launch_bounds__(kBlock) void sorted_check_kernel(const uint32_t *__restrict__ sorted, size_t n_sorted,
                                                              const uint32_t *__restrict__ unsorted, size_t n,
                                                              const uint8_t *__restrict__ cls, size_t n_text,
                                                              const uint32_t *__restrict__ blank_bits) {
  __shared__ uint32_t acc[7];
  if (threadIdx.x < 7) acc[threadIdx.x] = 0u;
  __syncthreads();
  uint32_t bad = 0, cnt[2] = {0, 0}, sum[2] = {0, 0}, x[2] = {0, 0};
  const size_t first = static_cast<size_t>(blockIdx.x) * kBlock + threadIdx.x, stride = static_cast<size_t>(gridDim.x) * kBlock;
  for (size_t i = first; i < n_sorted; i += stride) {
    const uint32_t k = sorted[i];
    if (i + 1 < n_sorted && k > sorted[i + 1]) bad++;
    if (blank_bits && key_is_blank(blank_bits, k)) bad++;
    cnt[0]++;
    sum[0] += k;
    x[0] ^= k;
  }
  for (size_t i = first; i < n; i += stride) {
    if (blank_bits && i < n_text && (cls[i] & kClsSpace)) continue;
    const uint32_t k = unsorted[i];
    cnt[1]++;
    sum[1] += k;
    x[1] ^= k;
  }
  if (bad) atomicAdd(&acc[6], bad);
  for (int s = 0; s < 2; s++) {
    if (cnt[s]) {
      atomicAdd(&acc[3 * s], cnt[s]);
      atomicAdd(&acc[3 * s + 1], sum[s]);
      atomicXor(&acc[3 * s + 2], x[s]);
    }
  }
  __syncthreads();
  if (threadIdx.x < 6 && acc[threadIdx.x]) {
    if (threadIdx.x % 3 == 2) {
      atomicXor(&g_wp_sorted_sig[threadIdx.x], acc[threadIdx.x]);
    } else {
      atomicAdd(&g_wp_sorted_sig[threadIdx.x], acc[threadIdx.x]);
    }
  }
  if (threadIdx.x == 6 && acc[6]) atomicAdd(&g_wp_oob[kSiteSortOrder], acc[6]);
}
__global__ void sorted_check_close_kernel() {
  bool same = true;
  for (int j = 0; j < 3; j++) same = same && g_wp_sorted_sig[j] == g_wp_sorted_sig[3 + j];
  wp_in_bounds(same, kSiteSortOrder);
  for (int j = 0; j < 6; j++) g_wp_sorted_sig[j] = 0u;
}
#endif

template <typename SymT>
struct LinearPath {
  const wp_vocab *v;
  Context *c;
  EncodeStats &S;
  Arena &ar, &aa;
  const uint8_t *d_text;
  size_t nbytes;
  const uint32_t *d_tile_prefix;
  size_t n_text, n;
  uint32_t *d_cps;
  uint8_t *d_cls;
  int bits;
  bool text_only;
  int offs_unit;
  RowsCall *rows;
  const NormMap *nmap;

  hipStream_t st, st2;
  const HostVocab &hv;
  bool full, prune, use_trie, key_lookup, keys_only, window_store, use_digit_bytes, staged_possible, sparse_emit;
  bool early_refine;
  bool wide_ran = false;
  uint32_t need_depth;
  int M, P, P_cap, bucket_shift, bucket_shift_all, key_shift, key_shift_all, hb_n, win_mid;
  unsigned sl_tiles, sl_groups, nbuckets, nbuckets_all, nkbuckets, nkbuckets_all;
  size_t radix_words, emit_tiles, walk_blocks, claim_size, list_cap;

  SymT *d_sym = nullptr, *d_vsym = nullptr;
  Key0 *KA = nullptr, *KB = nullptr;
  uint32_t *VA = nullptr, *VB = nullptr;
  uint32_t *X0 = nullptr, *X1 = nullptr;
  uint8_t *DG0 = nullptr, *DG1 = nullptr;
  RankEntry *d_rank = nullptr;
  uint32_t *d_node_of_slot = nullptr;
  int32_t *d_lcp = nullptr;
  uint32_t *d_sa = nullptr, *d_gdepth = nullptr;
  RankEntry *d_hd_n = nullptr;
  int32_t *d_emit = nullptr, *d_dbg_best = nullptr;
  uint32_t *d_anchors = nullptr, *d_anchor_cnt = nullptr, *d_anchor_tmp = nullptr, *d_emit_cnt = nullptr, *d_emit_tmp = nullptr,
           *d_blk_cnt = nullptr, *d_blk_off = nullptr, *d_tile_scratch = nullptr;
  uint32_t *AS0 = nullptr, *AS1 = nullptr, *AG = nullptr, *AD0 = nullptr, *AD1 = nullptr, *LA = nullptr, *LB = nullptr, *d_tdep = nullptr;
  uint64_t *LK0 = nullptr, *LK1 = nullptr, *LK2 = nullptr;
  uint32_t *LV0 = nullptr, *LV1 = nullptr, *LPOS = nullptr;
  uint32_t *d_ghead = nullptr, *d_gneed0 = nullptr, *d_gneed1 = nullptr, *d_lg_head = nullptr, *d_lg_off = nullptr;
  RerankAgg *d_agg = nullptr, *d_chunk_agg = nullptr;
  uint32_t *d_claim = nullptr, *d_claim_need = nullptr, *d_gclaim = nullptr, *d_gfirst = nullptr, *d_gdep = nullptr, *d_gnode = nullptr,
           *d_gdone = nullptr, *d_rng_lo = nullptr, *d_rng_hi = nullptr, *d_child_sym = nullptr, *d_radix_tmp = nullptr,
           *d_radix_tmp2 = nullptr;
  uint8_t *d_rng_long = nullptr;
  uint32_t *d_mslot0 = nullptr, *d_mslot1 = nullptr, *d_midx0 = nullptr, *d_midx1 = nullptr, *d_minfo = nullptr, *d_tile_mlo = nullptr;
  int32_t *d_mid = nullptr, *d_rf = nullptr, *d_rb = nullptr, *d_cover_f = nullptr, *d_cover_b = nullptr;
  int32_t *d_tmin_f = nullptr, *d_tmin_b = nullptr, *d_gmin_f = nullptr, *d_gmin_b = nullptr, *d_pval_p = nullptr, *d_pval_s = nullptr;
  uint32_t *d_ps0 = nullptr, *d_ps1 = nullptr, *d_pv0 = nullptr, *d_pv1 = nullptr, *d_bidx = nullptr;
  int2 *d_bfast = nullptr, *d_bfast_all = nullptr;
  uint32_t *d_bidx_all = nullptr;
  uint32_t *d_gend = nullptr, *d_kstart = nullptr, *d_kbidx = nullptr, *d_kbidx_all = nullptr;
  int32_t *d_kval_p = nullptr, *d_kval_s = nullptr;
  int2 *d_kbfast = nullptr, *d_kbfast_all = nullptr;
  unsigned long long *d_cand_table = nullptr;
  uint32_t *d_cand_filter = nullptr, *d_cand_lo = nullptr, *d_cand_hi = nullptr, *d_gcand = nullptr;
  uint32_t *d_tok_group = nullptr;
  uint32_t *d_cand_bcnt = nullptr, *d_cand_boff = nullptr, *d_cand_scan = nullptr;
  int cand_bits = 0;
  uint32_t *d_blank_bits = nullptr;
  uint2 *d_ospill = nullptr, *d_cspan = nullptr, *d_offs = nullptr;
  uint32_t *d_byte_of = nullptr;
  long long *d_line_starts = nullptr, *d_row_splits = nullptr;
  uint32_t *d_row_base = nullptr;

  SymbolCode code;
  DevCode dcode{};
  DigitBytes db;
  RadixPlan sort_plan;
  bool hist_in_keys = false;
  bool drop_blanks = false;
  size_t n_sorted = 0;
  int cur = 0, rounds = 1;
  Key0 *keys = nullptr, *other_keys = nullptr;
  uint32_t *vals = nullptr, *other_vals = nullptr, *slots = nullptr, *other_slots = nullptr, *adep = nullptr, *other_dep = nullptr;
  uint32_t *avals = nullptr, *spare_vals = nullptr;
  bool classified = false, anchors_queued = false;
  size_t n_act = 0, n_large = 0, n_large_groups = 0, n_groups = 0;
  StepTable steps{}, steps_all{};
  StepTable ksteps{}, ksteps_all{};
  CandSet cand{};
  CandRuns cand_runs{};
  size_t n_cand = 0;

  LinearPath(const wp_vocab *v_, Context *c_, EncodeStats &S_, Arena &ar_, Arena &aa_, const uint8_t *text, size_t nb,
             const uint32_t *tile_prefix, size_t n_text_, size_t n_, uint32_t *cps, uint8_t *cls, int bits_, bool text_only_,
             int offs_unit_, RowsCall *rows_ = nullptr, const NormMap *nmap_ = nullptr)
      : v(v_), c(c_), S(S_), ar(ar_), aa(aa_), d_text(text), nbytes(nb), d_tile_prefix(tile_prefix), n_text(n_text_), n(n_),
        d_cps(cps), d_cls(cls), bits(bits_), text_only(text_only_), offs_unit(offs_unit_), rows(rows_), nmap(nmap_), st(c_->stream), st2(c_->stream2),
        hv(v_->hv) {
    full = v->full_depth || hv.n_dup_eligible > 0 || v->lcp_kasai;
    need_depth = static_cast<uint32_t>(std::min<int64_t>(hv.longest + 1, 0x7fffffff));
    M = static_cast<int>(hv.elig_id.size());
    prune = !full && (M > 0 || text_only);
    use_trie = text_only && !full && M > 0;
    key_lookup = use_trie && !v->keep_debug && kKeyBits <= 32;
    keys_only = key_lookup && !v->indexed_round0 && sizeof(SymT) == 1;
    early_refine = keys_only && !v->late_refine;
    sl_tiles = cdiv(n, kSlTile);
    sl_groups = cdiv(sl_tiles, kSlGroup);
    P = kStepsPerMark * M + 1;
    P_cap = P + 2 * M + 2;
    const int bucket_bits = std::min(kStepBucketBitsMax, std::max(kStepBucketBits, bit_length(4 * static_cast<size_t>(P))));
    bucket_shift = std::max(0, bit_length(n) - bucket_bits);
    nbuckets = static_cast<unsigned>(((n - 1) >> bucket_shift) + 1);
    bucket_shift_all = std::max(0, bit_length(n) - kStepBucketBits);
    nbuckets_all = static_cast<unsigned>(((n - 1) >> bucket_shift_all) + 1);
    const int kb = std::min(kKeyBits, std::max(1, bit_length(n - 1) - bucket_shift));
    const int kb_all = std::min(kKeyBits, std::max(1, bit_length(n - 1) - bucket_shift_all));
    key_shift = kKeyBits - kb;
    key_shift_all = kKeyBits - kb_all;
    nkbuckets = 1u << kb;
    nkbuckets_all = 1u << kb_all;
    radix_words = std::max(radix_tmp_words<uint64_t>(n), radix_tmp_words<uint32_t>(std::max<size_t>(n, static_cast<size_t>(P_cap))));
    emit_tiles = cdiv(std::max<size_t>(n_text, 1), kScanTile);
    walk_blocks = cdiv(std::max<size_t>(n_text, 1), kBlock);
    sparse_emit = v->sparse_emit || EnvOptions::get().sparse_emit;
    staged_possible = !sparse_emit && !v->cover_anchors && hv.soft.empty();
    use_digit_bytes = n > kRadixSmallN;
    claim_size = 1024;
    while (claim_size < 2 * static_cast<size_t>(std::max(M, 1))) claim_size *= 2;
    cand_bits = bit_length(claim_size - 1);
    hb_n = bit_length(n - 1);
    window_store = n >= (1u << 22);
    win_mid = hb_n - kWinBits <= kRadixBits ? hb_n : kWinBits + (hb_n - kWinBits + 1) / 2;
    if (!prune) {
      list_cap = n;
    } else {
      const size_t guess = c->list_hint ? c->list_hint : n / 8;
      list_cap = std::min(n, guess + guess / 4 + 65536);
    }
    S.symbol_bits = bits;
    S.full_depth = full;
    S.trie_refine = use_trie ? 1 : 0;
    S.key_bits = kKeyBits;
    S.round0_keys_only = keys_only ? 1 : 0;
    S.round0_candidates = keys_only ? 0 : -1;
    n_sorted = n;
    S.round0_sorted = static_cast<int64_t>(n);
  }

  void fork() {
    WP_HIP(hipEventRecord(c->evs[kEvFork], st));
    WP_HIP(hipStreamWaitEvent(st2, c->evs[kEvFork], 0));
  }
  void join() {
    WP_HIP(hipEventRecord(c->evs[kEvJoin], st2));
    WP_HIP(hipStreamWaitEvent(st, c->evs[kEvJoin], 0));
  }

  void plan() {
    const bool ref = !text_only;
    const bool want_lcp = ref || v->keep_debug;
    const size_t lc = list_cap, lg = lc / 2 + static_cast<size_t>(M) + 8;
    const size_t rr_tiles_l = cdiv(lc, kRrTile);
    const size_t rtiles = cdiv(std::max<size_t>(n_text, 1), kReachTile);
    for (int pass = 0; pass < 2; pass++) {
      d_sym = ar.take<SymT>(n + 16);
      KA = ar.take<Key0>(n + 16);
      KB = ar.take<Key0>(n + 16);
      VA = ar.take<uint32_t>(n + 16);
      VB = ar.take<uint32_t>(n + 16);
      X0 = ar.take<uint32_t>(n + 16);
      X1 = ar.take<uint32_t>(n + 16);
      DG0 = use_digit_bytes ? ar.take<uint8_t>(n + 64) : nullptr;
      DG1 = use_digit_bytes ? ar.take<uint8_t>(n + 64) : nullptr;
      d_rank = ar.take<RankEntry>(n);
      d_node_of_slot = use_trie ? ar.take<uint32_t>(n) : nullptr;
      d_lcp = want_lcp ? ar.take<int32_t>(n) : nullptr;
      d_sa = (v->keep_debug || v->lcp_kasai) ? ar.take<uint32_t>(n) : nullptr;
      d_gdepth = (use_trie && !want_lcp) ? nullptr : ar.take<uint32_t>(n);
      d_hd_n = (want_lcp || !prune) ? ar.take<RankEntry>(n + 16) : nullptr;
      d_dbg_best = v->keep_debug ? ar.take<int32_t>(2 * n) : nullptr;
      d_emit = ar.take<int32_t>(n_text + 1);
      d_anchors = ar.take<uint32_t>(n_text + 1);
      d_anchor_cnt = ar.take<uint32_t>(emit_tiles + 1);
      d_anchor_tmp = ar.take<uint32_t>(cdiv(emit_tiles, kScanTile) + 8);
      d_emit_cnt = ar.take<uint32_t>(emit_tiles + 1);
      d_emit_tmp = ar.take<uint32_t>(cdiv(walk_blocks, kScanTile) + 8);
      d_blk_cnt = ar.take<uint32_t>(walk_blocks + 2);
      d_blk_off = ar.take<uint32_t>(walk_blocks + 2);
// ... 22 lines not shown
      d_radix_tmp = ar.take<uint32_t>(radix_words);
      d_radix_tmp2 = use_trie ? ar.take<uint32_t>(std::max(radix_tmp_words<uint64_t>(lc), keys_only ? radix_tmp_words<uint32_t>(n) : 0))
                              : nullptr;
      d_claim = ar.take<uint32_t>(claim_size);
      if (keys_only) {
        uint32_t *zeroed = ar.take<uint32_t>(3 * claim_size);
        d_cand_lo = zeroed;
        d_cand_hi = zeroed ? zeroed + claim_size : nullptr;
        d_claim_need = zeroed ? zeroed + 2 * claim_size : nullptr;
      } else {
        d_claim_need = ar.take<uint32_t>(claim_size);
      }
      d_gclaim = ar.take<uint32_t>(M + 4);
      d_gfirst = ar.take<uint32_t>(M + 4);
      d_gdep = ar.take<uint32_t>(M + 4);
      d_gnode = ar.take<uint32_t>(M + 4);
      d_gdone = ar.take<uint32_t>(M + 4);
      d_rng_lo = ar.take<uint32_t>(M + 1);
      d_rng_hi = ar.take<uint32_t>(M + 1);
      d_rng_long = ar.take<uint8_t>(M + 1);
      d_vsym = use_trie ? ar.take<SymT>(hv.stream.size() + 16) : nullptr;
      d_child_sym = use_trie ? ar.take<uint32_t>(hv.lt_child_cp.size() + 1) : nullptr;
      d_mslot0 = ar.take<uint32_t>(M + 1);
      d_mslot1 = ar.take<uint32_t>(M + 1);
      d_midx0 = ar.take<uint32_t>(M + 1);
      d_midx1 = ar.take<uint32_t>(M + 1);
      d_mid = ar.take<int32_t>(M + 1);
      d_minfo = ar.take<uint32_t>(M + 1);
      d_rf = ar.take<int32_t>(M + 1);
      d_cover_f = ar.take<int32_t>(2 * static_cast<size_t>(M) + 2);
      d_cover_b = ar.take<int32_t>(2 * static_cast<size_t>(M) + 2);
      d_rb = ar.take<int32_t>(M + 1);
      d_tile_mlo = ref ? ar.take<uint32_t>(sl_tiles + 2) : nullptr;
      d_tmin_f = ref ? ar.take<int32_t>(sl_tiles + 1) : nullptr;
      d_tmin_b = ref ? ar.take<int32_t>(sl_tiles + 1) : nullptr;
      d_gmin_f = ref ? ar.take<int32_t>(sl_groups + 1) : nullptr;
      d_gmin_b = ref ? ar.take<int32_t>(sl_groups + 1) : nullptr;
      d_ps0 = ar.take<uint32_t>(P_cap + 1);
      d_ps1 = ar.take<uint32_t>(P_cap + 1);
      d_pv0 = ar.take<uint32_t>(P_cap + 1);
      d_pv1 = ar.take<uint32_t>(P_cap + 1);
      d_pval_p = ar.take<int32_t>(P_cap + 1);
      d_pval_s = ar.take<int32_t>(P_cap + 1);
      d_bidx = ar.take<uint32_t>(static_cast<size_t>(nbuckets) + 2);
      d_bfast = ar.take<int2>(static_cast<size_t>(nbuckets) + 1);
      d_bidx_all = bucket_shift_all != bucket_shift ? ar.take<uint32_t>(static_cast<size_t>(nbuckets_all) + 2) : nullptr;
      d_bfast_all = bucket_shift_all != bucket_shift ? ar.take<int2>(static_cast<size_t>(nbuckets_all) + 1) : nullptr;
      d_gend = key_lookup ? ar.take<uint32_t>(M + 4) : nullptr;
      d_kstart = key_lookup ? ar.take<uint32_t>(P_cap + 1) : nullptr;
      d_kval_p = key_lookup ? ar.take<int32_t>(P_cap + 1) : nullptr;
      d_kval_s = key_lookup ? ar.take<int32_t>(P_cap + 1) : nullptr;
      d_kbidx = key_lookup ? ar.take<uint32_t>(static_cast<size_t>(nkbuckets) + 2) : nullptr;
      d_kbfast = key_lookup ? ar.take<int2>(static_cast<size_t>(nkbuckets) + 1) : nullptr;
      d_kbidx_all = (key_lookup && key_shift_all != key_shift) ? ar.take<uint32_t>(static_cast<size_t>(nkbuckets_all) + 2) : nullptr;
      d_kbfast_all = (key_lookup && key_shift_all != key_shift) ? ar.take<int2>(static_cast<size_t>(nkbuckets_all) + 1) : nullptr;
      d_cand_table = keys_only ? ar.take<unsigned long long>(claim_size) : nullptr;
      d_cand_filter = keys_only ? ar.take<uint32_t>(kCandFilterWords) : nullptr;
      d_gcand = keys_only ? ar.take<uint32_t>(M + 4) : nullptr;
      d_tok_group = keys_only ? ar.take<uint32_t>(M + 1) : nullptr;
      d_cand_bcnt = keys_only ? ar.take<uint32_t>(cdiv(n, kKeyTile) + 2) : nullptr;
      d_cand_boff = keys_only ? ar.take<uint32_t>(cdiv(n, kKeyTile) + 2) : nullptr;
      d_cand_scan = keys_only ? ar.take<uint32_t>(cdiv(cdiv(n, kKeyTile), kScanTile) + 8) : nullptr;
      d_blank_bits = keys_only ? ar.take<uint32_t>(kBlankWords) : nullptr;
      const bool offs = offs_unit >= 0;
      d_ospill = offs ? ar.take<uint2>(n_text + 16) : nullptr;
      d_cspan = offs ? ar.take<uint2>(n_text + 16) : nullptr;
      d_offs = offs ? ar.take<uint2>(n_text + 1) : nullptr;
      d_byte_of = ((offs_unit == WP_OFFSETS_BYTES && !nmap) || rows) ? ar.take<uint32_t>(n_text + 1) : nullptr;
      d_line_starts = (rows && (!rows->d_doc_off || nmap)) ? ar.take<long long>(rows->n_rows + 1) : nullptr;
      d_row_splits = rows ? ar.take<long long>(rows->n_rows + 1) : nullptr;
      d_row_base = (rows && rows->unit >= 0) ? ar.take<uint32_t>(rows->n_rows + 1) : nullptr;
      if (pass == 0) ar.commit();
    }
    ar.arm(st);
  }

  void launch_anchors(hipStream_t as) {
    anchors_queued = true;
    const unsigned atiles = cdiv(n_text, kAnchorTile);
    if (!staged_possible) WP_HIP(hipMemsetAsync(d_emit, 0x80, n_text * sizeof(int32_t), as));
    hipLaunchKernelGGL(anchor_count_kernel, dim3(atiles), dim3(kBlock), 0, as, d_cls, static_cast<const uint8_t *>(nullptr),
                       n_text, d_anchor_cnt);
    device_exclusive_scan(d_anchor_cnt, d_anchor_cnt, atiles, d_anchor_tmp, c->d_scalars + kScalarAnchors, as);
    hipLaunchKernelGGL(anchor_write_kernel, dim3(atiles), dim3(kBlock), 0, as, d_cls, static_cast<const uint8_t *>(nullptr),
                       n_text, d_anchor_cnt, d_anchors);
    hipLaunchKernelGGL(anchor_gap_kernel, dim3(std::min<size_t>(atiles, 1024)), dim3(kBlock), 0, as, d_anchors,
                       c->d_scalars + kScalarAnchors, n_text, d_cls, hv.soft.empty() ? 1 : 0, c->d_scalars + kScalarAnchorGap);
  }

  void symbols_and_keys() {
    const int lo_bits = sizeof(SymT) == 1 ? 0 : std::max(0, bits - 8);
    constexpr int kCodeReuse = 64;
    const bool reuse_code = c->code_cached && c->code_alphabet == static_cast<uint32_t>(S.alphabet) && c->code_bits == bits &&
                            c->code_lo == lo_bits && c->code_uses < kCodeReuse;
    if (!reuse_code) WP_HIP(hipMemsetAsync(c->d_symhist, 0, sizeof(uint32_t) * 256, st));
    constexpr uint32_t kBlankCpRuns[3][2] = {{0x09, 7}, {0x20, 2}, {kSpaceToken, 2}};
    uint32_t h_blank_lut[3][7] = {};
    hipLaunchKernelGGL(HIP_KERNEL_NAME(decode_write_kernel<SymT>), dim3(cdiv(nbytes, kDecTile)), dim3(kBlock), 0, st, d_text,
                       nbytes, d_tile_prefix, c->d_lut, d_sym, d_cls, d_cps, c->d_cls_bmp, c->d_soft,
                       static_cast<int>(hv.soft.size()), reuse_code ? nullptr : c->d_symhist, lo_bits);
    hipLaunchKernelGGL(HIP_KERNEL_NAME(map_vocab_symbols_kernel<SymT>), dim3(cdiv(n - n_text, kBlock)), dim3(kBlock), 0, st,
                       c->d_stream, n_text, n, c->d_lut, d_sym);
    if (reuse_code) {
      code = c->code_cache;
      c->code_uses++;
    } else {
      std::vector<uint32_t> h32(256);
      WP_HIP(hipMemcpyAsync(h32.data(), c->d_symhist, sizeof(uint32_t) * 256, hipMemcpyDeviceToHost, st));
      if (sizeof(SymT) == 1) {
        for (int r = 0; r < 3; r++) {
          WP_HIP(hipMemcpyAsync(h_blank_lut[r], c->d_lut + kBlankCpRuns[r][0], sizeof(uint32_t) * kBlankCpRuns[r][1],
                                hipMemcpyDeviceToHost, st));
        }
      }
      WP_HIP(hipStreamSynchronize(st));
      const size_t nitems = (static_cast<size_t>(S.alphabet) >> lo_bits) + 1;
      std::vector<uint64_t> freq(nitems);
      for (size_t i = 0; i < nitems; i++) freq[i] = h32[i];
      code = build_symbol_code(freq, bits, true);
      if (!code.uniform_bits) {
        code.lo_bits = lo_bits;
        code.avg_bits += lo_bits;
      }
      c->code_cache = code;
      c->code_cached = true;
      c->code_alphabet = static_cast<uint32_t>(S.alphabet);
      c->code_bits = bits;
      c->code_lo = lo_bits;
      c->code_uses = 0;
      uint64_t all = 0, blank = 0;
      for (size_t i = 0; i < nitems; i++) all += freq[i];
      if (sizeof(SymT) == 1) {
        for (int r = 0; r < 3; r++) {
          for (uint32_t k = 0; k + 1 < kBlankCpRuns[r][1]; k++) {
            const uint32_t cp = kBlankCpRuns[r][0] + k, s = h_blank_lut[r][k] + 1u;
            if (is_space(cp) && h_blank_lut[r][k + 1] != h_blank_lut[r][k] && s < nitems) blank += freq[s];
          }
        }
      }
      c->code_blank_share = all ? static_cast<double>(blank) / static_cast<double>(all) : 0.0;
      if (!code.uniform_bits) {
        const size_t blob_bytes = 512 + 256 + kDecodeTableBytes;
        std::memset(c->h_code, 0, blob_bytes);
        std::memcpy(c->h_code, code.cw.data(), code.cw.size() * sizeof(uint16_t));
        std::memcpy(c->h_code + 512, code.len.data(), code.len.size());
        std::memcpy(c->h_code + 768, code.bmask.data(), kDecodeTableBytes);
        WP_HIP(hipMemcpyAsync(c->d_code, c->h_code, blob_bytes, hipMemcpyHostToDevice, st));
      }
    }
    dcode = DevCode{reinterpret_cast<const uint16_t *>(c->d_code), c->d_code + 512, c->d_code + 768,
                    code.uniform_bits ? code.uniform_bits : -code.lo_bits};
    S.symbols_per_key = static_cast<int32_t>(kKeyBits / std::max(1.0, code.avg_bits));
    if (keys_only) {
      WP_HIP(hipMemsetAsync(d_cand_table, 0, claim_size * sizeof(unsigned long long), st));
      WP_HIP(hipMemsetAsync(d_cand_filter, 0, kCandFilterWords * sizeof(uint32_t), st));
      hipLaunchKernelGGL(long_key_set_kernel, dim3(cdiv(static_cast<size_t>(M) * kWave, kBlock)), dim3(kBlock), 0, st, c->d_stream,
                         c->d_elig_start, c->d_elig_info, M, c->d_lut, dcode, d_cand_table, cand_bits, d_cand_filter);
      cand.filter = d_cand_filter;
      cand.table = d_cand_table;
      cand.table_bits = cand_bits;
      cand.slot = VA;
      cand.pos = VB;
      cand.bcount = d_cand_bcnt;
    }
    size_t cand_blocks = 0;
    int min_len = code.uniform_bits ? code.uniform_bits : 99;
    for (uint8_t l : code.len) min_len = std::min<int>(min_len, l);
    if (sizeof(SymT) == 1 && min_len >= kKeys8MinLen) {
      cand.tile = kKeys8Tile;
      cand_blocks = cdiv(n, kKeys8Tile);
// ... 569 lines not shown
    if (key_shift_all != key_shift) {
      hipLaunchKernelGGL(piece_bucket_kernel, dim3(cdiv(nkbuckets_all + 1, kBlock)), dim3(kBlock), 0, st, d_kstart, P, key_shift_all,
                         nkbuckets_all, d_kbidx_all);
      hipLaunchKernelGGL(piece_bucket_fast_kernel, dim3(cdiv(nkbuckets_all, kBlock)), dim3(kBlock), 0, st, d_kbidx_all, d_kval_p,
                         d_kval_s, nkbuckets_all, d_kbfast_all);
      ksteps_all = StepTable{d_kstart, d_kval_p, d_kval_s, d_kbidx_all, key_shift_all, pack_steps, d_kbfast_all};
    }
    WP_LAUNCH_CHECK();
  }

  void walk_long_words(const WalkArgs &wa, size_t n_anchors) {
    const uint32_t lw_cap = static_cast<uint32_t>(n_text / kMaxAnchorGap + 2);
    LongWord *d_lw = reinterpret_cast<LongWord *>(d_tile_scratch);
    uint32_t *d_lw_off = d_tile_scratch + 2 * static_cast<size_t>(lw_cap);
    uint32_t *d_lw_fail = d_lw_off + lw_cap + 1;
    hipLaunchKernelGGL(long_word_collect_kernel, dim3(std::min<size_t>(cdiv(std::max<size_t>(n_anchors, 1), kBlock), 2048)),
                       dim3(kBlock), 0, st, d_anchors, c->d_scalars + kScalarAnchors, n_text, d_cls, d_lw, lw_cap, c->d_scalars + kScalarLongWords);
    WP_LAUNCH_CHECK();
    fetch_scalars(c, kScalarLongWords);
    const uint32_t nw = std::min(c->h_scalars[kScalarLongWords], lw_cap);
    if (nw == 0) return;
    S.walk.n_long_words = static_cast<int64_t>(nw);
    std::vector<LongWord> h_lw(nw);
    WP_HIP(hipMemcpyAsync(h_lw.data(), d_lw, sizeof(LongWord) * nw, hipMemcpyDeviceToHost, st));
    WP_HIP(hipStreamSynchronize(st));
    std::vector<uint32_t> h_off(nw + 1);
    uint64_t total64 = 0;
    uint32_t longest = 0;
    for (uint32_t i = 0; i < nw; i++) {
      h_off[i] = static_cast<uint32_t>(total64);
      total64 += h_lw[i].end - h_lw[i].begin;
      longest = std::max(longest, h_lw[i].end - h_lw[i].begin);
    }
    h_off[nw] = static_cast<uint32_t>(total64);
    const uint32_t total = static_cast<uint32_t>(total64);
    WP_HIP(hipMemcpyAsync(d_lw_off, h_off.data(), sizeof(uint32_t) * (nw + 1), hipMemcpyHostToDevice, st));
    WP_HIP(hipMemsetAsync(d_lw_fail, 0, sizeof(uint32_t) * nw, st));
    int32_t *d_lid = reinterpret_cast<int32_t *>(VA);
    uint32_t *jump_a = X1, *jump_b = X0;
    uint8_t *d_mark = reinterpret_cast<uint8_t *>(KB);
    const dim3 grid(cdiv(total, kBlock));
    WalkArgs wa_all = wa;
    wa_all.steps = steps_all;
    wa_all.ksteps = ksteps_all;
    hipLaunchKernelGGL(long_word_next_kernel, grid, dim3(kBlock), 0, st, wa_all, d_lw, d_lw_off, nw, total, d_lid, jump_a, d_mark);
    WP_HIP(hipStreamSynchronize(st));
    for (uint32_t reach = 1; reach < longest; reach *= 2) {
      hipLaunchKernelGGL(long_word_mark_kernel, grid, dim3(kBlock), 0, st, jump_a, total, d_mark);
      hipLaunchKernelGGL(long_word_double_kernel, grid, dim3(kBlock), 0, st, jump_a, total, jump_b);
      std::swap(jump_a, jump_b);
    }
    hipLaunchKernelGGL(long_word_mark_kernel, grid, dim3(kBlock), 0, st, jump_a, total, d_mark);
    hipLaunchKernelGGL(long_word_fail_kernel, grid, dim3(kBlock), 0, st, d_lid, d_mark, d_lw_off, nw, total, d_lw_fail);
    if (offs_unit >= 0) {
      uint32_t *d_lw_end = d_lw_fail + lw_cap;
      WP_HIP(hipMemsetAsync(d_lw_end, 0xff, sizeof(uint32_t) * nw, st));
      hipLaunchKernelGGL(long_word_end_kernel, grid, dim3(kBlock), 0, st, d_lw, d_lw_off, nw, total, d_lid, d_lw_end);
      hipLaunchKernelGGL(HIP_KERNEL_NAME(long_word_emit_kernel<true>), grid, dim3(kBlock), 0, st, wa, d_lw, d_lw_off, nw, total, d_lid,
                         d_mark, d_lw_fail, d_ospill, static_cast<const uint32_t *>(d_lw_end));
    } else {
      hipLaunchKernelGGL(HIP_KERNEL_NAME(long_word_emit_kernel<false>), grid, dim3(kBlock), 0, st, wa, d_lw, d_lw_off, nw, total, d_lid,
                         d_mark, d_lw_fail, static_cast<uint2 *>(nullptr), static_cast<const uint32_t *>(nullptr));
    }
    WP_LAUNCH_CHECK();
    S.anchor_mode = 2;
  }

  size_t cover_anchors(WalkArgs &wa) {
    uint32_t *d_reach = VA, *d_reach_tiles = d_tile_scratch;
    uint8_t *d_aflags = reinterpret_cast<uint8_t *>(X1);
    const unsigned rtiles = cdiv(n_text, kReachTile), atiles = cdiv(n_text, kAnchorTile);
    uint32_t *d_wp_tiles = d_reach_tiles + rtiles + 1;
    uint32_t *d_ns_tiles = d_wp_tiles + rtiles + 1;
    uint32_t *d_gap_a = d_ns_tiles + rtiles + 1, *d_gap_b = d_gap_a + rtiles + 1;
    hipLaunchKernelGGL(gap_tiles_kernel, dim3(cdiv(rtiles, kBlock)), dim3(kBlock), 0, st, d_anchors, c->d_scalars + kScalarAnchors, n_text, rtiles,
                       v->cover_anchors ? 1 : 0, d_gap_a, d_gap_b);
    hipLaunchKernelGGL(reach_kernel, dim3(rtiles), dim3(kBlock), 0, st, wa, d_reach, d_reach_tiles, d_gap_a, d_gap_b);
    hipLaunchKernelGGL(reach_spine_kernel, dim3(1), dim3(1024), 0, st, d_reach_tiles, static_cast<size_t>(rtiles));
    WP_HIP(hipMemsetAsync(d_anchor_cnt, 0, sizeof(uint32_t) * atiles, st));
    hipLaunchKernelGGL(cover_flags_kernel, dim3(rtiles), dim3(kBlock), 0, st, d_cls, d_reach, d_reach_tiles, n_text, d_aflags,
                       d_wp_tiles, d_ns_tiles, d_gap_a, d_gap_b, d_anchor_cnt);
    hipLaunchKernelGGL(suffix_min_kernel, dim3(2), dim3(1024), 0, st, d_wp_tiles, d_ns_tiles, static_cast<size_t>(rtiles));
    device_exclusive_scan(d_anchor_cnt, d_anchor_cnt, atiles, d_anchor_tmp, c->d_scalars + kScalarAnchors, st);
    hipLaunchKernelGGL(anchor_write_kernel, dim3(atiles), dim3(kBlock), 0, st, d_cls, d_aflags, n_text, d_anchor_cnt, d_anchors);
    WP_LAUNCH_CHECK();
    fetch_scalars(c, kScalarAnchors);
    wa.aflags = d_aflags;
    wa.wp_from_tile = d_wp_tiles;
    wa.ns_from_tile = d_ns_tiles;
    S.anchor_mode = 1;
    return c->h_scalars[kScalarAnchors];
  }

  int32_t *walk(size_t *n_ids_out) {
    int32_t *d_ids = reinterpret_cast<int32_t *>(VB);
    *n_ids_out = 0;
    if (n_text == 0) return d_ids;
    WalkArgs wa{d_cls, n_text, d_rank, steps, c->d_tok_len, hv.unk_id, d_emit, nullptr, nullptr, nullptr,
                hv.soft.empty() ? 1 : 0, static_cast<int32_t>(hv.tokens.size()),
                key_lookup ? reinterpret_cast<const uint32_t *>(KA) : nullptr, ksteps, drop_blanks ? 1 : 0};
    S.anchor_mode = 0;
    join();
    fetch_scalars(c, kScalarAnchorGap);
    size_t n_anchors = c->h_scalars[kScalarAnchors];
    const size_t max_anchor_gap = c->h_scalars[kScalarAnchorGap];
    S.walk.max_anchor_gap = static_cast<int32_t>(max_anchor_gap);
    const bool all_hard = hv.soft.empty();
    bool staged = staged_possible && max_anchor_gap <= kMaxAnchorGap;
    if (staged_possible && !staged) WP_HIP(hipMemsetAsync(d_emit, 0x80, n_text * sizeof(int32_t), st));
    if (!v->cover_anchors && all_hard && max_anchor_gap > kMaxAnchorGap) {
      walk_long_words(wa, n_anchors);
    } else if (v->cover_anchors || max_anchor_gap > kMaxAnchorGap) {
      n_anchors = cover_anchors(wa);
      staged = !sparse_emit;
    }
    S.n_anchors = static_cast<int64_t>(n_anchors);
    const size_t acap = std::max<size_t>(n_anchors, 1);
    const bool offs = offs_unit >= 0;
    if (staged) {
      int32_t *d_ctmp = reinterpret_cast<int32_t *>(X0);
      const unsigned sblocks = cdiv(acap, static_cast<size_t>(kWbWords));
      if (S.anchor_mode == 0 && all_hard && max_anchor_gap > kWideMin) {
        uint32_t *d_wide_list = reinterpret_cast<uint32_t *>(KB), *d_wide_cnt = VA;
        wide_ran = true;
        clear_scalars(c, kScalarWideWords, kScalarWideWords, st);
        hipLaunchKernelGGL(wide_collect_kernel, dim3(std::min<size_t>(cdiv(acap, kBlock), 2048)), dim3(kBlock), 0, st, d_anchors,
                           c->d_scalars + kScalarAnchors, n_text, d_wide_list, c->d_scalars + kScalarWideWords);
        WalkArgs wa_all = wa;
        wa_all.steps = steps_all;
        wa_all.ksteps = ksteps_all;
        const dim3 wgrid(std::min<size_t>(cdiv(acap, kBlock / kWave), 8192));
        if (offs) {
          hipLaunchKernelGGL(HIP_KERNEL_NAME(walk_wide_kernel<true>), wgrid, dim3(kBlock), 0, st, wa_all, d_anchors, c->d_scalars + kScalarAnchors,
                             d_wide_list, c->d_scalars + kScalarWideWords, d_wide_cnt, d_ospill);
          hipLaunchKernelGGL(HIP_KERNEL_NAME(walk_lean_kernel<true, true>), dim3(sblocks), dim3(kBlock), 0, st, wa, d_anchors,
                             c->d_scalars + kScalarAnchors, acap, d_ctmp, d_blk_cnt, d_wide_cnt, d_ospill, d_cspan);
        } else {
          hipLaunchKernelGGL(HIP_KERNEL_NAME(walk_wide_kernel<false>), wgrid, dim3(kBlock), 0, st, wa_all, d_anchors, c->d_scalars + kScalarAnchors,
                             d_wide_list, c->d_scalars + kScalarWideWords, d_wide_cnt, static_cast<uint2 *>(nullptr));
          hipLaunchKernelGGL(HIP_KERNEL_NAME(walk_lean_kernel<true, false>), dim3(sblocks), dim3(kBlock), 0, st, wa, d_anchors,
                             c->d_scalars + kScalarAnchors, acap, d_ctmp, d_blk_cnt, d_wide_cnt, static_cast<uint2 *>(nullptr),
                             static_cast<uint2 *>(nullptr));
        }
      } else if (offs) {
        hipLaunchKernelGGL(HIP_KERNEL_NAME(walk_lean_kernel<false, true>), dim3(sblocks), dim3(kBlock), 0, st, wa, d_anchors,
                           c->d_scalars + kScalarAnchors, acap, d_ctmp, d_blk_cnt, static_cast<const uint32_t *>(nullptr), d_ospill, d_cspan);
      } else {
        hipLaunchKernelGGL(HIP_KERNEL_NAME(walk_lean_kernel<false, false>), dim3(sblocks), dim3(kBlock), 0, st, wa, d_anchors,
                           c->d_scalars + kScalarAnchors, acap, d_ctmp, d_blk_cnt, static_cast<const uint32_t *>(nullptr),
                           static_cast<uint2 *>(nullptr), static_cast<uint2 *>(nullptr));
      }
      device_exclusive_scan(d_blk_cnt, d_blk_off, sblocks, d_emit_tmp, c->d_scalars + kScalarIds, st);
      if (offs) {
        hipLaunchKernelGGL(HIP_KERNEL_NAME(emit_gather_kernel<true>), dim3(sblocks), dim3(kBlock), 0, st, d_anchors, c->d_scalars + kScalarAnchors,
                           acap, d_ctmp, d_blk_cnt, d_blk_off, d_ids, kWbWords, static_cast<const uint2 *>(d_cspan), d_offs);
      } else {
        hipLaunchKernelGGL(HIP_KERNEL_NAME(emit_gather_kernel<false>), dim3(sblocks), dim3(kBlock), 0, st, d_anchors, c->d_scalars + kScalarAnchors,
                           acap, d_ctmp, d_blk_cnt, d_blk_off, d_ids, kWbWords, static_cast<const uint2 *>(nullptr),
                           static_cast<uint2 *>(nullptr));
      }
    } else {
      if (offs) {
        hipLaunchKernelGGL(HIP_KERNEL_NAME(walk_kernel<true>), dim3(cdiv(acap, kBlock)), dim3(kBlock), 0, st, wa, d_anchors,
                           c->d_scalars + kScalarAnchors, acap, d_ospill);
      } else {
        hipLaunchKernelGGL(HIP_KERNEL_NAME(walk_kernel<false>), dim3(cdiv(acap, kBlock)), dim3(kBlock), 0, st, wa, d_anchors,
                           c->d_scalars + kScalarAnchors, acap, static_cast<uint2 *>(nullptr));
      }
      const unsigned tiles = cdiv(n_text, kScanTile);
      hipLaunchKernelGGL(emit_count_kernel, dim3(tiles), dim3(kBlock), 0, st, d_emit, n_text, d_emit_cnt);
      device_exclusive_scan(d_emit_cnt, d_emit_cnt, tiles, d_emit_tmp, c->d_scalars + kScalarIds, st);
      if (offs) {
        hipLaunchKernelGGL(HIP_KERNEL_NAME(emit_write_kernel<true>), dim3(tiles), dim3(kBlock), 0, st, d_emit, n_text, d_emit_cnt, d_ids,
                           static_cast<const uint2 *>(d_ospill), d_offs);
      } else {
        hipLaunchKernelGGL(HIP_KERNEL_NAME(emit_write_kernel<false>), dim3(tiles), dim3(kBlock), 0, st, d_emit, n_text, d_emit_cnt, d_ids,
                           static_cast<const uint2 *>(nullptr), static_cast<uint2 *>(nullptr));
      }
    }
    S.staged_emit = staged ? 1 : 0;
    S.walk.lean = staged ? 1 : 0;
    WP_LAUNCH_CHECK();
    return d_ids;
  }

  void row_structure(size_t n_ids) {
    const size_t n_rows = rows->n_rows;
    const long long *d_starts = rows->d_doc_off;
    if (!d_starts) {
      if (nmap) hipLaunchKernelGGL(norm_fill_starts_kernel, dim3(cdiv(n_rows + 1, kBlock)), dim3(kBlock), 0, st, d_line_starts, n_rows + 1, static_cast<long long>(nbytes));
      hipLaunchKernelGGL(line_write_kernel, dim3(cdiv(nbytes, kLineTile)), dim3(kBlock), 0, st, d_text, nbytes,
                         static_cast<const uint32_t *>(rows->d_line_cnt), n_rows, d_line_starts);
      d_starts = d_line_starts;
    }
    if (n_ids > 0) {
      hipLaunchKernelGGL(cp_byte_kernel, dim3(cdiv(nbytes, kDecTile)), dim3(kBlock), 0, st, d_text, nbytes, d_tile_prefix, n_text,
                         d_byte_of);
      if (nmap && rows->d_doc_off) {
        hipLaunchKernelGGL(norm_doc_starts_kernel, dim3(cdiv(n_rows + 1, kBlock)), dim3(kBlock), 0, st, rows->d_doc_off, n_rows, *nmap,
                           static_cast<const uint32_t *>(d_byte_of), nbytes, d_line_starts);
        d_starts = d_line_starts;
      }
      hipLaunchKernelGGL(row_splits_kernel, dim3(cdiv(n_rows + 1, kBlock)), dim3(kBlock), 0, st, d_starts, n_rows,
                         static_cast<const uint32_t *>(d_byte_of), n_text, static_cast<const uint2 *>(d_offs), n_ids, rows->unit,
                         d_row_splits, d_row_base);
      if (nmap && d_row_base) {
        hipLaunchKernelGGL(norm_row_base_kernel, dim3(cdiv(n_rows + 1, kBlock)), dim3(kBlock), 0, st, d_starts, n_rows,
                           static_cast<const uint32_t *>(d_byte_of), n_text, *nmap, rows->unit, d_row_base);
      }
    } else {
      WP_HIP(hipMemsetAsync(d_row_splits, 0, (n_rows + 1) * sizeof(long long), st));
    }
    WP_LAUNCH_CHECK();
    rows->d_starts = d_starts;
    rows->d_row_splits = d_row_splits;
  }

  void finish(int32_t *d_ids, size_t *n_ids_out) {
    c->d_offs = nullptr;
    if (offs_unit >= 0 && n_text > 0) {
      fetch_scalars(c, kScalarIds);
      const size_t n_ids = c->h_scalars[kScalarIds];
      if (rows) row_structure(n_ids);
      if (nmap) {
        if (n_ids > 0 && (!rows || rows->unit >= 0)) {
          hipLaunchKernelGGL(span_source_kernel, dim3(cdiv(n_ids, kBlock)), dim3(kBlock), 0, st, d_offs, n_ids, *nmap, offs_unit);
          WP_LAUNCH_CHECK();
        }
      } else if (offs_unit == WP_OFFSETS_BYTES && n_ids > 0) {
        if (!rows) {
          hipLaunchKernelGGL(cp_byte_kernel, dim3(cdiv(nbytes, kDecTile)), dim3(kBlock), 0, st, d_text, nbytes, d_tile_prefix, n_text,
                             d_byte_of);
        }
// ... 258 lines not shown
```

### wordpiece_amd/csrc/scanline.h

```cpp
#pragma once
#include "primitives.h"
#include "suffix_array.h"

namespace wp {

constexpr int kSlItems = 16;
constexpr int kSlTile = kBlock * kSlItems;
constexpr int32_t kLcpInf = 0x7fffffff;
constexpr uint32_t kMarkLenMask = 0x0fffffffu;
#ifndef WP_STEP_BUCKET_BITS
#define WP_STEP_BUCKET_BITS 18
#endif
constexpr int kStepBucketBits = WP_STEP_BUCKET_BITS;
#ifndef WP_STEP_BUCKET_BITS_MAX
#define WP_STEP_BUCKET_BITS_MAX 21
#endif
constexpr int kStepBucketBitsMax = WP_STEP_BUCKET_BITS_MAX;
constexpr int kStepIdBits = 20;
constexpr int kStepMaxLen = 1 << 11;
constexpr uint32_t kMarkSurvBwd = 1u << 28;
constexpr uint32_t kMarkSurvFwd = 1u << 29;
constexpr int kMarkClsShift = 30;

__device__ __forceinline__ int32_t boundary_lcp(const int32_t *__restrict__ lcp, size_t n, long long x) {
// ... 335 lines not shown
    const int q = base + lane;
    bool cover = false;
    int cls = 0;
    if (q < mv.M) {
      const uint32_t info = mv.minfo[q];
      cls = static_cast<int>(info >> kMarkClsShift);
      cover = mv.reach_bwd[q] < static_cast<int32_t>(slot);
    }
#pragma unroll
    for (int c = 0; c < 2; c++) {
      const uint64_t b = __ballot(cover && cls == c);
      if (yq[c] < 0 && b) yq[c] = base + __ffsll(static_cast<long long>(b)) - 1;
    }
  }
  if (lane < 2) {
    const int c = lane;
    const int x = c ? xq[1] : xq[0], y = c ? yq[1] : yq[0];
    int wq = -1;
    if (x >= 0 && y >= 0) {
      const int32_t xl = static_cast<int32_t>(mv.minfo[x] & kMarkLenMask), yl = static_cast<int32_t>(mv.minfo[y] & kMarkLenMask);
      wq = xl > yl ? x : y;
    } else if (x >= 0) {
      wq = x;
    } else if (y >= 0) {
      wq = y;
    }
    int32_t r = wq >= 0 ? mv.mid[wq] : -1;
    if (packed && r >= 0) r |= static_cast<int32_t>(mv.minfo[wq] & kMarkLenMask) << kStepIdBits;
    (c ? pval_suffix : pval_prefix)[k] = r;
  }
}

__global__ __launch_bounds__(kBlock) void piece_bucket_kernel(const uint32_t *__restrict__ pstart, int P, int shift,
                                                              unsigned nbuckets, uint32_t *__restrict__ bidx) {
  const unsigned b = blockIdx.x * kBlock + threadIdx.x;
  if (b > nbuckets) return;
  const uint64_t key = static_cast<uint64_t>(b) << shift;
  int lo = 0, hi = P;
  while (lo < hi) {
    const int md = (lo + hi) >> 1;
    if (pstart[md] < key) lo = md + 1; else hi = md;
  }
  bidx[b] = static_cast<uint32_t>(lo);
}

constexpr int32_t kStepSlow = static_cast<int32_t>(0x80000000u);
constexpr int32_t kStepNeeded = -2;
__global__ __launch_bounds__(kBlock) void piece_bucket_fast_kernel(const uint32_t *__restrict__ bidx,
                                                                   const int32_t *__restrict__ pval_prefix,
                                                                   const int32_t *__restrict__ pval_suffix, unsigned nbuckets,
                                                                   int2 *__restrict__ bfast) {
  const unsigned b = blockIdx.x * kBlock + threadIdx.x;
  if (b >= nbuckets) return;
  const uint32_t lo = bidx[b], hi = bidx[b + 1];
  bfast[b] = lo == hi ? int2{pval_prefix[lo - 1], pval_suffix[lo - 1]}
                      : int2{kStepSlow | static_cast<int32_t>(hi - lo), static_cast<int32_t>(lo)};
}

struct StepTable {
  const uint32_t *pstart;
  const int32_t *pval_prefix, *pval_suffix;
  const uint32_t *bidx;
  int shift;
  int packed;
  const int2 *bfast;
};
__device__ __forceinline__ int32_t step_id(const StepTable &st, int32_t raw) {
  return (st.packed && raw >= 0) ? (raw & ((1 << kStepIdBits) - 1)) : raw;
}
__device__ __forceinline__ int32_t step_len(const StepTable &st, int32_t raw, const int32_t *__restrict__ tok_len) {
  return st.packed ? (raw >> kStepIdBits) : tok_len[raw];
}

__device__ __forceinline__ int step_lookup(const StepTable &st, uint32_t r) {
  const uint32_t b = r >> st.shift;
  int lo = static_cast<int>(st.bidx[b]), hi = static_cast<int>(st.bidx[b + 1]);
  while (lo < hi) {
    const int md = (lo + hi) >> 1;
    if (st.pstart[md] <= r) lo = md + 1; else hi = md;
  }
  return lo - 1;
}

__device__ __forceinline__ int32_t step_raw(const StepTable &st, uint32_t r, bool prefix) {
  const int2 e = st.bfast[r >> st.shift];
  if (e.x >= kStepNeeded) return prefix ? e.x : e.y;
  const int n = e.x & 0x7fffffff;
  int lo = e.y, hi = e.y + n;
  while (lo < hi) {
    const int md = (lo + hi) >> 1;
    if (st.pstart[md] <= r) lo = md + 1; else hi = md;
  }
  return prefix ? st.pval_prefix[lo - 1] : st.pval_suffix[lo - 1];
}


__global__ __launch_bounds__(kBlock) void group_starts_kernel(const uint32_t *__restrict__ gfirst,
                                                              const uint32_t *__restrict__ ghead,
                                                              const uint32_t *__restrict__ totals, size_t n,
                                                              uint32_t *__restrict__ pstart_tail, uint32_t *__restrict__ gend) {
  const uint32_t g = blockIdx.x * kBlock + threadIdx.x;
  if (g >= totals[1]) return;
  const uint32_t f = gfirst[g], e = f + (ghead[g + 1] - ghead[g]);
  const uint32_t last = static_cast<uint32_t>(n - 1);
  pstart_tail[2 * static_cast<size_t>(g)] = f;
  pstart_tail[2 * static_cast<size_t>(g) + 1] = min(e, last);
  gend[g] = e;
}

__global__ __launch_bounds__(kBlock) void key_steps_kernel(const uint32_t *__restrict__ pstart, const int32_t *__restrict__ pval_prefix,
                                                           const int32_t *__restrict__ pval_suffix, int P,
                                                           const uint32_t *__restrict__ sorted_keys, uint32_t *__restrict__ kstart,
                                                           int32_t *__restrict__ kval_prefix, int32_t *__restrict__ kval_suffix) {
  const int k = blockIdx.x * kBlock + threadIdx.x;
  if (k >= P) return;
  kstart[k] = k == 0 ? 0u : sorted_keys[pstart[k]];
  kval_prefix[k] = pval_prefix[k];
  kval_suffix[k] = pval_suffix[k];
}

__device__ __forceinline__ int starts_lower_bound(const uint32_t *__restrict__ pstart, int P, uint32_t x) {
  int lo = 0, hi = P;
  while (lo < hi) {
    const int md = (lo + hi) >> 1;
    if (pstart[md] < x) lo = md + 1; else hi = md;
  }
  return lo;
}

__global__ __launch_bounds__(kBlock) void key_steps_needed_kernel(const uint32_t *__restrict__ gfirst,
                                                                  const uint32_t *__restrict__ gend, uint32_t n_groups,
                                                                  const uint32_t *__restrict__ pstart, int P,
                                                                  int32_t *__restrict__ kval_prefix, int32_t *__restrict__ kval_suffix) {
  const uint32_t g = blockIdx.x * kBlock + threadIdx.x;
  if (g >= n_groups) return;
  const int k0 = starts_lower_bound(pstart, P, gfirst[g]), k1 = starts_lower_bound(pstart, P, gend[g]);
  for (int k = k0; k < k1; k++) {
    kval_prefix[k] = kStepNeeded;
    kval_suffix[k] = kStepNeeded;
  }
}

__global__ __launch_bounds__(kBlock) void key_steps_check_kernel(const uint32_t *__restrict__ pstart, int P,
                                                                 const uint32_t *__restrict__ sorted_keys,
                                                                 const int32_t *__restrict__ kval_prefix,
                                                                 const int32_t *__restrict__ kval_suffix) {
  const int k = blockIdx.x * kBlock + threadIdx.x;
  if (k == 0 || k >= P) return;
  const uint32_t s = pstart[k];
  if (s == 0 || kval_prefix[k] == kStepNeeded || sorted_keys[s - 1] != sorted_keys[s]) return;
  wp_in_bounds(kval_prefix[k] == kval_prefix[k - 1] && kval_suffix[k] == kval_suffix[k - 1], kSiteKeyStep);
}

__global__ __launch_bounds__(kBlock) void step_expand_kernel(StepTable st, size_t n, int32_t *__restrict__ best_prefix,
                                                             int32_t *__restrict__ best_suffix) {
  const size_t x = static_cast<size_t>(blockIdx.x) * kBlock + threadIdx.x;
  if (x >= n) return;
  const int k = step_lookup(st, static_cast<uint32_t>(x));
  best_prefix[x] = step_id(st, st.pval_prefix[k]);
  best_suffix[x] = step_id(st, st.pval_suffix[k]);
}

}
```

### wordpiece_amd/csrc/walk.h

```cpp
#pragma once
#include <type_traits>

#include "primitives.h"
#include "scanline.h"
#include "suffix_array.h"

namespace wp {

constexpr int kReachTile = kBlock * 8;
constexpr size_t kMaxAnchorGap = 2048;
constexpr int32_t kNoEmit = static_cast<int32_t>(0x80808080u);

struct WalkArgs {
  const uint8_t *cls;
  size_t n_text;
  const RankEntry *rank;
  StepTable steps;
  const int32_t *tok_len;
  int32_t unk_id;
  int32_t *emit;
  const uint8_t *aflags;
  const uint32_t *wp_from_tile;
  const uint32_t *ns_from_tile;
  int all_hard;
  int32_t n_tokens;
  const uint32_t *pkey;
  StepTable ksteps;
  int blanks_dropped;
};

__device__ __forceinline__ void check_blank_lookup(const WalkArgs &a, uint8_t cls) {
#ifdef WP_DEBUG_BOUNDS
  if (a.blanks_dropped) wp_in_bounds(!(cls & kClsSpace), kSiteBlankLookup);
#else
  (void)a;
  (void)cls;
#endif
}

__device__ __forceinline__ int32_t step_value_of(const WalkArgs &a, uint32_t key, uint32_t r, bool prefix) {
  if (a.pkey) {
    const int32_t v = step_raw(a.ksteps, key, prefix);
    if (v != kStepNeeded) return v;
  }
  return step_raw(a.steps, r, prefix);
}
__device__ __forceinline__ uint32_t step_key(const WalkArgs &a, size_t q) { return a.pkey ? a.pkey[q] : 0u; }
__device__ __forceinline__ int32_t step_value(const WalkArgs &a, size_t q, bool prefix) {
  check_blank_lookup(a, a.cls[q]);
  const uint32_t key = step_key(a, q);
  const uint32_t r = rank_of(a.rank[q]);
  return step_value_of(a, key, r, prefix);
}

__device__ __forceinline__ bool w_space(const WalkArgs &a, size_t p) { return a.cls[p] & kClsSpace; }
__device__ __forceinline__ bool w_word_prefix(const WalkArgs &a, size_t p) {
  return p == 0 || (a.cls[p] & kClsSpacing) || (a.cls[p - 1] & kClsSpacing);
}
__device__ __forceinline__ bool w_hard(uint8_t c) { return (c & kClsSpacing) && !(c & kClsSoft); }
__device__ __forceinline__ bool w_anchor(const WalkArgs &a, size_t p) {
  if (a.aflags) return a.aflags[p] != 0;
  const uint8_t c = a.cls[p];
  if (c & kClsSpace) return false;
  return p == 0 || w_hard(c) || w_hard(a.cls[p - 1]);
}

constexpr int kStageIds = 4;

struct SparseOut {
  int32_t *emit;
  const int32_t *tok_len;
  __device__ __forceinline__ void push(size_t p, int32_t id) { emit[p] = id; }
  __device__ __forceinline__ void word_start() {}
  __device__ __forceinline__ void rollback(size_t since, size_t p) {
    size_t q = since;
    while (q < p) {
      const int32_t t = emit[q];
      emit[q] = kNoEmit;
      q += static_cast<size_t>(tok_len[t]);
    }
  }
};

struct StagedOut {
  int32_t *stage;
  int32_t *spill;
  uint32_t c = 0, mark = 0;
  uint32_t stride = kBlock;
  __device__ __forceinline__ void push(size_t, int32_t id) {
    if (c < static_cast<uint32_t>(kStageIds)) {
      stage[c * stride] = id;
    } else {
      spill[c] = id;
    }
    c++;
  }
  __device__ __forceinline__ void word_start() { mark = c; }
  __device__ __forceinline__ void rollback(size_t, size_t) { c = mark; }
  __device__ __forceinline__ int32_t get(uint32_t j) const {
    return j < static_cast<uint32_t>(kStageIds) ? stage[j * stride] : spill[j];
  }
};

template <typename Out>
struct OutSpans {
  static constexpr bool value = false;
};

struct SparseSpanOut {
  int32_t *emit;
  const int32_t *tok_len;
// ... 127 lines not shown
    s.since = p;
    o.word_start();
  }
  return false;
}

template <typename Out>
__device__ __forceinline__ bool walk_step(const WalkArgs &a, WalkState &s, Out &o) {
  const StepWin W = step_window(a, s.p);
  check_blank_lookup(a, step_cb(a, W, s.p));
  const uint32_t key = step_key(a, s.p);
  const uint32_t r = rank_of(a.rank[s.p]);
  return walk_finish(a, s, o, W, step_value_of(a, key, r, step_word_prefix(a, W, s.p)));
}

template <typename Out>
__device__ inline void walk_from(const WalkArgs &a, size_t p, Out &o) {
  WalkState s{p, p};
  o.word_start();
  while (s.p < a.n_text) {
    if (walk_step(a, s, o)) return;
  }
}

constexpr int kAnchorBytes = 16;
constexpr int kAnchorTile = kBlock * kAnchorBytes;

__device__ __forceinline__ uint32_t anchor_mask16(const uint8_t *__restrict__ cls, const uint8_t *__restrict__ aflags,
                                                  size_t n, size_t i) {
  if (i >= n) return 0u;
  uint32_t w[4];
  if (aflags) cls = aflags;
  if (i + kAnchorBytes <= n) {
    const uint4 v = *reinterpret_cast<const uint4 *>(cls + i);
    w[0] = v.x;
    w[1] = v.y;
    w[2] = v.z;
    w[3] = v.w;
  } else {
#pragma unroll
    for (int q = 0; q < 4; q++) {
      w[q] = 0;
#pragma unroll
      for (int j = 0; j < 4; j++) {
        const size_t p = i + 4 * q + j;
        if (p < n) w[q] |= static_cast<uint32_t>(cls[p]) << (8 * j);
      }
    }
  }
  uint32_t valid = 0xffffu;
  if (i + kAnchorBytes > n) valid = (1u << (n - i)) - 1u;
  if (aflags) {
    uint32_t m = 0;
#pragma unroll
    for (int q = 0; q < 4; q++) m |= (((w[q] & 0x01010101u) * 0x01020408u) >> 24) << (4 * q);
    return m & valid;
  }
  uint32_t space = 0, hard = 0;
#pragma unroll
  for (int q = 0; q < 4; q++) {
    const uint32_t sp = w[q] & 0x01010101u;
    const uint32_t hd = (w[q] >> 1) & ~(w[q] >> 2) & 0x01010101u;
    space |= ((sp * 0x01020408u) >> 24) << (4 * q);
    hard |= ((hd * 0x01020408u) >> 24) << (4 * q);
  }
  uint32_t before = 1u;
  if (i > 0) before = w_hard(cls[i - 1]) ? 1u : 0u;
  return ~space & (hard | (hard << 1) | before) & valid;
}

__global__ __launch_bounds__(kBlock) void anchor_count_kernel(const uint8_t *__restrict__ cls,
                                                              const uint8_t *__restrict__ aflags, size_t n,
                                                              uint32_t *__restrict__ tile_counts) {
  __shared__ uint32_t sm[8];
  const size_t i = static_cast<size_t>(blockIdx.x) * kAnchorTile + static_cast<size_t>(threadIdx.x) * kAnchorBytes;
  const uint32_t c = __popc(anchor_mask16(cls, aflags, n, i));
  uint32_t tot;
  (void)block_excl_sum(c, sm, tot);
  if (threadIdx.x == 0) tile_counts[blockIdx.x] = tot;
}

__global__ __launch_bounds__(kBlock) void anchor_write_kernel(uint8_t *__restrict__ cls, const uint8_t *__restrict__ aflags,
                                                              size_t n, const uint32_t *__restrict__ tile_prefix,
                                                              uint32_t *__restrict__ anchors) {
  __shared__ uint32_t sm[8];
  const size_t i = static_cast<size_t>(blockIdx.x) * kAnchorTile + static_cast<size_t>(threadIdx.x) * kAnchorBytes;
  uint32_t m = anchor_mask16(cls, aflags, n, i);
  if (i < n) {
    uint32_t w[4] = {0, 0, 0, 0};
    const int cnt = static_cast<int>(min(static_cast<size_t>(kAnchorBytes), n - i));
    if (cnt == kAnchorBytes) {
      const uint4 v = *reinterpret_cast<const uint4 *>(cls + i);
      w[0] = v.x;
      w[1] = v.y;
      w[2] = v.z;
      w[3] = v.w;
    } else {
      for (int j = 0; j < cnt; j++) w[j >> 2] |= static_cast<uint32_t>(cls[i + j]) << (8 * (j & 3));
    }
    uint32_t spc = 0;
#pragma unroll
    for (int q = 0; q < 4; q++) spc |= ((((w[q] >> 1) & 0x01010101u) * 0x01020408u) >> 24) << (4 * q);
    const uint32_t before = i == 0 ? 1u : ((cls[i - 1] & kClsSpacing) ? 1u : 0u);
    const uint32_t wp = (spc | (spc << 1) | before) & 0xffffu;
#pragma unroll
    for (int q = 0; q < 4; q++) {
      const uint32_t wq = (((wp >> (4 * q)) & 15u) * 0x00204081u) & 0x01010101u;
      const uint32_t aq = (((m >> (4 * q)) & 15u) * 0x00204081u) & 0x01010101u;
      w[q] = (w[q] & 0x0f0f0f0fu) | (wq << 4) | (aq << 5);
    }
    if (cnt == kAnchorBytes) {
      *reinterpret_cast<uint4 *>(cls + i) = uint4{w[0], w[1], w[2], w[3]};
    } else {
      for (int j = 0; j < cnt; j++) cls[i + j] = static_cast<uint8_t>(w[j >> 2] >> (8 * (j & 3)));
    }
  }
  uint32_t tot;
  uint32_t o = tile_prefix[blockIdx.x] + block_excl_sum(static_cast<uint32_t>(__popc(m)), sm, tot);
  while (m) {
    const int j = __ffs(static_cast<int>(m)) - 1;
    m &= m - 1;
    anchors[o++] = static_cast<uint32_t>(i + j);
  }
}

__global__ __launch_bounds__(kBlock) void anchor_gap_kernel(const uint32_t *__restrict__ anchors,
                                                            const uint32_t *__restrict__ n_anchors_dev, size_t n_text,
                                                            const uint8_t *__restrict__ cls, int all_hard,
                                                            uint32_t *__restrict__ max_gap) {
  __shared__ int32_t sm[8];
  const size_t na = *n_anchors_dev;
  uint32_t g = 0;
  for (size_t k = static_cast<size_t>(blockIdx.x) * kBlock + threadIdx.x; k <= na;
       k += static_cast<size_t>(gridDim.x) * kBlock) {
    const uint32_t hi = k < na ? anchors[k] : static_cast<uint32_t>(n_text);
    const uint32_t lo = k > 0 ? anchors[k - 1] : 0u;
    uint32_t d = hi - lo;
    if (d > kMaxAnchorGap && all_hard) {
      uint32_t q = lo;
      const uint32_t stop = min(hi, lo + static_cast<uint32_t>(kMaxAnchorGap) + 1u);
      while (q < stop && !(cls[q] & kClsSpace)) q++;
      d = q - lo;
    }
    g = max(g, d);
  }
  const int32_t m = -block_reduce_min(-static_cast<int32_t>(g), sm);
  if (threadIdx.x == 0 && m > 0) atomicMax(max_gap, static_cast<uint32_t>(m));
}

static_assert(kReachTile <= static_cast<int>(kMaxAnchorGap), "a tile meets at most two long gaps");
__global__ __launch_bounds__(kBlock) void gap_tiles_kernel(const uint32_t *__restrict__ anchors,
                                                           const uint32_t *__restrict__ n_anchors_dev, size_t n_text,
                                                           unsigned tiles, int all, uint32_t *__restrict__ gap_a_end,
                                                           uint32_t *__restrict__ gap_b_start) {
  const unsigned t = blockIdx.x * kBlock + threadIdx.x;
  if (t >= tiles) return;
  const uint32_t t0 = t * static_cast<uint32_t>(kReachTile);
  const uint32_t t1 = static_cast<uint32_t>(min(static_cast<size_t>(t0) + kReachTile, n_text));
  if (all) {
    gap_a_end[t] = t1;
    gap_b_start[t] = t0;
    return;
  }
  const uint32_t na = *n_anchors_dev;
  auto gap_of = [&](uint32_t p, uint32_t &lo, uint32_t &hi) {
    uint32_t a = 0, b = na;
    while (a < b) {
      const uint32_t md = (a + b) >> 1;
      if (anchors[md] <= p) a = md + 1; else b = md;
    }
    lo = a ? anchors[a - 1] : 0u;
    hi = a < na ? anchors[a] : static_cast<uint32_t>(n_text);
  };
  uint32_t lo, hi;
  gap_of(t0, lo, hi);
  gap_a_end[t] = hi - lo > kMaxAnchorGap ? min(hi, t1) : t0;
  gap_of(t1 - 1, lo, hi);
  gap_b_start[t] = hi - lo > kMaxAnchorGap ? max(lo, t0) : t1;
}

__global__ __launch_bounds__(kBlock) void reach_kernel(WalkArgs a, uint32_t *__restrict__ reach,
                                                       uint32_t *__restrict__ tile_max,
                                                       const uint32_t *__restrict__ gap_a_end,
                                                       const uint32_t *__restrict__ gap_b_start) {
  __shared__ int32_t sm[8];
  const size_t base = static_cast<size_t>(blockIdx.x) * kReachTile;
  {
    const uint32_t t0 = static_cast<uint32_t>(base);
    const uint32_t t1 = static_cast<uint32_t>(min(base + kReachTile, a.n_text));
    if (gap_a_end[blockIdx.x] <= t0 && gap_b_start[blockIdx.x] >= t1) {
      if (threadIdx.x == 0) tile_max[blockIdx.x] = 0u;
      return;
    }
  }
  uint32_t mx = 0;
#pragma unroll
  for (int j = 0; j < 8; j++) {
    const size_t q = base + static_cast<size_t>(j) * kBlock + threadIdx.x;
    if (q < a.n_text) {
      uint32_t r = static_cast<uint32_t>(q);
      if (!w_space(a, q)) {
// ... 479 lines not shown
            const int wq = w0 + u * kStride;
            const uint2 *ssrc = spans + (wq < WORDS ? wstart[wq] : 0u);
            uint2 *sdst = cspan + base + (wq < WORDS ? woff[wq] : 0u);
            for (uint32_t j = done + lane; j < min(c[u], done + kC * kWave); j += kWave) sdst[j] = ssrc[j];
          }
        }
        done += kC * kWave;
      }
    }
  }
  if (threadIdx.x == 0) blk_cnt[blockIdx.x] = tot;
}

constexpr int kWbPerWave = 256;
constexpr int kWbWords = kWbPerWave * (kBlock / kWave);
struct LinearStep {
  using State = WalkState;
  __device__ static __forceinline__ bool step(const WalkArgs &a, WalkState &s, StagedOut &o) { return walk_step(a, s, o); }
};

template <typename Args, typename Step, bool WIDE = false>
__global__ __launch_bounds__(kBlock) void walk_balanced_kernel(Args a, const uint32_t *__restrict__ anchors,
                                                               const uint32_t *__restrict__ n_anchors_dev, size_t cap,
                                                               int32_t *__restrict__ ctmp, uint32_t *__restrict__ blk_cnt,
                                                               const uint32_t *__restrict__ wide_cnt) {
  __shared__ int32_t stage[kStageIds * kWbWords];
  __shared__ uint32_t cnt[kWbWords];
  __shared__ uint32_t woff[WIDE ? kWbWords : 1], wstart[WIDE ? kWbWords : 1];
  __shared__ uint32_t sm[8];
  const int lane = lane_id(), w = wave_id();
  const size_t na = min(cap, static_cast<size_t>(*n_anchors_dev));
  const size_t a0 = static_cast<size_t>(blockIdx.x) * kWbWords;
  for (int q = threadIdx.x; q < kWbWords; q += kBlock) cnt[q] = 0;
  __syncthreads();
  const int wbase = w * kWbPerWave;
  int next = kWave;
  int widx = wbase + lane;
  bool active = a0 + static_cast<size_t>(widx) < na;
  typename Step::State s{0, 0};
  StagedOut o{stage + widx, a.emit, 0, 0, kWbWords};
  auto taken_wide = [&](int wd, uint32_t start) {
    if (!WIDE) return false;
    const size_t k = a0 + static_cast<size_t>(wd);
    const uint32_t hi = k + 1 < static_cast<size_t>(*n_anchors_dev) ? anchors[k + 1] : static_cast<uint32_t>(a.n_text);
    if (hi - start <= kWideMin) return false;
    cnt[wd] = wide_cnt[k];
    wstart[wd] = start;
    return true;
  };
  if (active) {
    const uint32_t start = anchors[a0 + widx];
    s = typename Step::State{start, start};
    o.spill = a.emit + start;
    if (taken_wide(widx, start)) active = false;
  }
  for (;;) {
    if (active) {
      const bool done = s.p >= a.n_text || Step::step(a, s, o);
      if (done) {
        cnt[widx] = o.c;
        active = false;
      }
    }
    const uint64_t idle = __ballot(!active);
    if (next < kWbPerWave) {
      if (!active) {
        const int cand = next + __popcll(idle & ((1ull << lane) - 1ull));
        if (cand < kWbPerWave && a0 + static_cast<size_t>(wbase + cand) < na) {
          widx = wbase + cand;
          const uint32_t start = anchors[a0 + widx];
          s = typename Step::State{start, start};
          o = StagedOut{stage + widx, a.emit + start, 0, 0, kWbWords};
          active = !taken_wide(widx, start);
        }
      }
      next += __popcll(idle);
    }
    if (!__ballot(active) && (!WIDE || next >= kWbPerWave)) break;
  }
  __syncthreads();
  assemble_word_lists<kWbWords, WIDE>(a.emit, anchors, a0, na, stage, cnt, sm, ctmp, blk_cnt, woff, wstart);
}

template <bool WIDE, bool OFFS = false>
__global__ __launch_bounds__(kBlock) void walk_lean_kernel(WalkArgs a, const uint32_t *__restrict__ anchors,
                                                           const uint32_t *__restrict__ n_anchors_dev, size_t cap,
                                                           int32_t *__restrict__ ctmp, uint32_t *__restrict__ blk_cnt,
                                                           const uint32_t *__restrict__ wide_cnt, uint2 *__restrict__ spans,
                                                           uint2 *__restrict__ cspan) {
  using Out = typename std::conditional<OFFS, StagedSpanOut, StagedOut>::type;
  __shared__ int32_t stage[kStageIds * kWbWords];
  __shared__ uint32_t cnt[kWbWords];
  __shared__ uint32_t woff[WIDE ? kWbWords : 1], wstart[WIDE ? kWbWords : 1];
  __shared__ uint32_t sm[8];
  const int lane = lane_id(), w = wave_id();
  const size_t na = min(cap, static_cast<size_t>(*n_anchors_dev));
  const size_t a0 = static_cast<size_t>(blockIdx.x) * kWbWords;
  const uint32_t end = static_cast<uint32_t>(a.n_text);
  for (int q = threadIdx.x; q < kWbWords; q += kBlock) cnt[q] = 0;
  __syncthreads();
  const int wbase = w * kWbPerWave;
  const int mine = a0 + static_cast<size_t>(wbase) < na
                       ? static_cast<int>(min(static_cast<size_t>(kWbPerWave), na - a0 - static_cast<size_t>(wbase)))
                       : 0;
  const bool stop_at_blank = !a.aflags && a.all_hard;
  int widx = wbase + lane;
  uint32_t p = 0, since = 0;
  Out o{stage + widx, a.emit, 0, 0, kWbWords};
  auto take = [&](int wd) {
    widx = wd;
    const size_t k = a0 + static_cast<size_t>(wd);
    const uint32_t start = anchors[k];
    p = since = start;
    o = Out{stage + wd, a.emit + start, 0, 0, kWbWords};
    if constexpr (OFFS) o.spans = spans + start;
    if (WIDE) {
      const uint32_t hi = k + 1 < static_cast<size_t>(*n_anchors_dev) ? anchors[k + 1] : end;
      if (hi - start > kWideMin) {
        cnt[wd] = wide_cnt[k];
        wstart[wd] = start;
        return false;
      }
    }
    return true;
  };
  bool active = lane < mine && take(wbase + lane);
  int next = min(kWave, mine);
  for (;;) {
    if (active) {
      bool done = true;
      if (p < end) {
        const uint32_t key = step_key(a, p);
        const uint32_t r = rank_of(a.rank[p]);
        uint32_t cw[4];
        __builtin_memcpy(cw, a.cls + p, 16);
        const int32_t raw = step_value_of(a, key, r, (cw[0] & kClsWordPrefix) != 0);
        check_blank_lookup(a, static_cast<uint8_t>(cw[0]));
        const int32_t id = step_id(a.steps, raw);
        bool fast = id >= 0 && wp_in_bounds(id < a.n_tokens, kSiteTokenId);
        uint32_t len = 0, p2 = 0, f = 0;
        if (fast) {
          len = static_cast<uint32_t>(step_len(a.steps, raw, a.tok_len));
          p2 = p + len;
          fast = len < 15 || p2 >= end;
        }
        if (fast && p2 < end) {
          const uint32_t d0 = len < 8 ? (len < 4 ? cw[0] : cw[1]) : (len < 12 ? cw[2] : cw[3]);
          f = __builtin_amdgcn_ubfe(d0, (len & 3u) * 8u, 8u);
          if (f & kClsSpace) {
            if (!stop_at_blank) {
              const uint32_t l1 = len + 1;
              const uint32_t d1 = l1 < 8 ? (l1 < 4 ? cw[0] : cw[1]) : (l1 < 12 ? cw[2] : cw[3]);
              const uint32_t f1 = __builtin_amdgcn_ubfe(d1, (l1 & 3u) * 8u, 8u);
              if (p2 + 1 < end && !(f1 & kClsSpace)) {
                p2 += 1;
                f = f1;
              } else {
                fast = p2 + 1 >= end;
                f = kClsAnchor;
                if (fast) p2 = end;
              }
            } else {
              f = kClsAnchor;
            }
          }
        }
        if (fast) {
          if constexpr (OFFS) {
            o.push_span(p, p + len, id);
          } else {
            o.push(p, id);
          }
          p = p2;
          done = p2 >= end || (f & kClsAnchor);
          if (!done && (f & kClsWordPrefix)) {
            since = p2;
            o.word_start();
          }
        } else {
          WalkState s{p, since};
          const StepWin W = step_window(a, p);
          done = walk_finish(a, s, o, W, raw);
          p = static_cast<uint32_t>(s.p);
          since = static_cast<uint32_t>(s.since);
        }
      }
      if (done) {
        cnt[widx] = o.c;
        active = false;
      }
    }
    const uint64_t idle = __ballot(!active);
    if (next < mine) {
      if (!active) {
        const int cand = next + __popcll(idle & ((1ull << lane) - 1ull));
        if (cand < mine) active = take(wbase + cand);
      }
      next = min(next + static_cast<int>(__popcll(idle)), mine);
    }
    if (!__ballot(active) && next >= mine) break;
  }
  __syncthreads();
  assemble_word_lists<kWbWords, WIDE, OFFS>(a.emit, anchors, a0, na, stage, cnt, sm, ctmp, blk_cnt, woff, wstart, spans, cspan);
}

template <bool OFFS = false>
__global__ __launch_bounds__(kBlock) void emit_gather_kernel(const uint32_t *__restrict__ anchors,
                                                             const uint32_t *__restrict__ n_anchors_dev, size_t cap,
                                                             const int32_t *__restrict__ ctmp,
                                                             const uint32_t *__restrict__ blk_cnt,
                                                             const uint32_t *__restrict__ blk_off,
                                                             int32_t *__restrict__ ids, int words,
                                                             const uint2 *__restrict__ cspan, uint2 *__restrict__ offs) {
  const size_t k0 = static_cast<size_t>(blockIdx.x) * words;
  if (k0 >= cap || k0 >= *n_anchors_dev) return;
  const size_t base = anchors[k0], off = blk_off[blockIdx.x];
  const uint32_t cnt = blk_cnt[blockIdx.x];
  for (uint32_t j = threadIdx.x; j < cnt; j += kBlock) ids[off + j] = ctmp[base + j];
  if (OFFS) {
    for (uint32_t j = threadIdx.x; j < cnt; j += kBlock) offs[off + j] = cspan[base + j];
  }
}

__global__ __launch_bounds__(kBlock) void emit_count_kernel(const int32_t *__restrict__ emit, size_t n,
                                                            uint32_t *__restrict__ tile_counts) {
  __shared__ uint32_t sm[8];
  const size_t base = static_cast<size_t>(blockIdx.x) * kScanTile;
  uint32_t c = 0;
#pragma unroll
  for (int j = 0; j < kScanItems; j++) {
    size_t i = base + static_cast<size_t>(j) * kBlock + threadIdx.x;
    if (i < n && emit[i] != kNoEmit) c++;
  }
  uint32_t tot;
  (void)block_excl_sum(c, sm, tot);
  if (threadIdx.x == 0) tile_counts[blockIdx.x] = tot;
}

template <bool OFFS = false>
__global__ __launch_bounds__(kBlock) void emit_write_kernel(const int32_t *__restrict__ emit, size_t n,
                                                            const uint32_t *__restrict__ tile_prefix,
                                                            int32_t *__restrict__ ids, const uint2 *__restrict__ spans,
                                                            uint2 *__restrict__ offs) {
  __shared__ uint32_t sm[8];
  const size_t base = static_cast<size_t>(blockIdx.x) * kScanTile + static_cast<size_t>(threadIdx.x) * kScanItems;
  int32_t v[kScanItems];
  uint32_t c = 0;
#pragma unroll
  for (int j = 0; j < kScanItems; j++) {
    size_t i = base + j;
    v[j] = i < n ? emit[i] : kNoEmit;
    c += v[j] != kNoEmit;
  }
  uint32_t tot;
  size_t o = static_cast<size_t>(block_excl_sum(c, sm, tot)) + tile_prefix[blockIdx.x];
#pragma unroll
  for (int j = 0; j < kScanItems; j++) {
    if (v[j] != kNoEmit) {
      if (OFFS) offs[o] = spans[base + j];
      ids[o++] = v[j];
    }
  }
}

}
```

Measured before the change: 31760.

## Defer rank loads in lean walk, mirror anchor scalars asynchronously, optional anchor key list

The lean walk kernel now looks up the key-step table first and loads the suffix rank only when the key lookup cannot resolve the step (late rank, on by default). This removes a dependent global load on most steps. The anchor count and max gap are copied to host on a side stream with an event, instead of a blocking fetch before the walk. An opt-in mode (options 2/3) also gathers each anchor's key during anchor writing so the walk can skip step_key, at the cost of extra key reads and an added stream wait.

After: 31730 (median of 3 runs). Within noise of the previous version (-0.1%).

```diff
diff --git a/include/wordpiece_amd.h b/include/wordpiece_amd.h
--- a/include/wordpiece_amd.h
+++ b/include/wordpiece_amd.h
@@ -139,6 +139,7 @@
 #define WP_NORM_STRIP_ACCENTS 4
 #define WP_NORM_BERT_UNCASED 7
 #define WP_OPT_LATE_REFINE 15
+#define WP_OPT_WALK_GATHER_KEYS  16
 int wp_set_option(wp_vocab *v, int option, int64_t value);
 
 int wp_normalize_cp(int flags, uint32_t cp, uint32_t out[3]);
@@ -210,6 +211,19 @@
   double ms_sort_to_scan;
 } wp_refine_sched;
 int wp_get_refine_sched(const wp_vocab *v, wp_refine_sched *out);
+#define WP_WALK_KEYS_LIST 0
+#define WP_WALK_KEYS_OPTION 1
+#define WP_WALK_KEYS_LAYOUT 2
+#define WP_WALK_KEYS_SMALL_TEXT 3
+#define WP_WALK_KEYS_SPARSE_WALK 4
+typedef struct {
+  int32_t from_list;
+  int32_t reason;
+  int32_t late_rank;
+  int32_t side_scalars;
+  int64_t capacity;
+} wp_walk_keys;
+int wp_get_walk_keys(const wp_vocab *v, wp_walk_keys *out);
 typedef struct {
   int64_t n_samples, n_out;
   int64_t n_cut;
diff --git a/wordpiece_amd/__init__.py b/wordpiece_amd/__init__.py
--- a/wordpiece_amd/__init__.py
+++ b/wordpiece_amd/__init__.py
@@ -14,6 +14,8 @@
 WP_OPT_SORT_BLANKS = 13
 WP_OPT_NORMALIZE = 14
 WP_OPT_LATE_REFINE = 15
+WP_OPT_WALK_GATHER_KEYS = 16
+WP_WALK_KEYS_LIST, WP_WALK_KEYS_OPTION, WP_WALK_KEYS_LAYOUT, WP_WALK_KEYS_SMALL_TEXT, WP_WALK_KEYS_SPARSE_WALK = 0, 1, 2, 3, 4
 WP_NORM_CLEAN, WP_NORM_LOWER, WP_NORM_STRIP_ACCENTS, WP_NORM_BERT_UNCASED = 1, 2, 4, 7
 WP_OFFSETS_BYTES, WP_OFFSETS_CODE_POINTS = 0, 1
 _OFFSET_UNITS = {"byte": WP_OFFSETS_BYTES, "char": WP_OFFSETS_CODE_POINTS}
@@ -31,7 +33,7 @@
     "wp_linear_encode_offsets", "wp_linear_encode_offsets_device",
     "wp_linear_encode_rows", "wp_linear_encode_rows_device", "wp_linear_encode_padded", "wp_linear_encode_padded_device",
     "wp_normalize_cp", "wp_normalize_device", "wp_normalize", "wp_get_norm_stats", "wp_get_walk_stats",
-    "wp_get_refine_stats", "wp_get_refine_sched",
+    "wp_get_refine_stats", "wp_get_refine_sched", "wp_get_walk_keys",
     "wp_linear_encode_inputs", "wp_linear_encode_inputs_device", "wp_get_inputs_stats",
     "wp_word_ids", "wp_word_ids_device", "wp_mlm_mask", "wp_mlm_mask_device", "wp_get_mask_stats",
     "wp_detokenize", "wp_detokenize_device", "wp_detok_piece", "wp_get_detok_stats",
@@ -84,6 +86,11 @@
 
 class RefineSched(C.Structure):
     _fields_ = [("early", C.c_int32), ("reserved", C.c_int32), ("ms_sort_to_scan", C.c_double)]
+
+
+class WalkKeys(C.Structure):
+    _fields_ = [("from_list", C.c_int32), ("reason", C.c_int32), ("late_rank", C.c_int32), ("side_scalars", C.c_int32),
+                ("capacity", C.c_int64)]
 
 
 class InputsSpec(C.Structure):
@@ -210,6 +217,8 @@
         L.wp_get_refine_stats.argtypes = [vp, C.POINTER(RefineStats)]
         if hasattr(L, "wp_get_refine_sched"):
             L.wp_get_refine_sched.argtypes = [vp, C.POINTER(RefineSched)]
+        if hasattr(L, "wp_get_walk_keys"):
+            L.wp_get_walk_keys.argtypes = [vp, C.POINTER(WalkKeys)]
         L.wp_linear_debug_fetch.argtypes = [vp, C.c_int, i32p, C.c_size_t, C.POINTER(C.c_size_t)]
         L.wp_free.argtypes = [vp]
         L.wp_free.restype = None
@@ -327,6 +336,11 @@
         rs = RefineSched()
         _check(lib().wp_get_refine_sched(self._h, C.byref(rs)))
         return {"early": int(rs.early), "ms_sort_to_scan": float(rs.ms_sort_to_scan)}
+
+    def walk_keys(self):
+        wk = WalkKeys()
+        _check(lib().wp_get_walk_keys(self._h, C.byref(wk)))
+        return {k: int(getattr(wk, k)) for k, _ in wk._fields_}
 
     def encode(self, text):
         b = _bytes(text)
diff --git a/wordpiece_amd/csrc/context.h b/wordpiece_amd/csrc/context.h
--- a/wordpiece_amd/csrc/context.h
+++ b/wordpiece_amd/csrc/context.h
@@ -24,12 +24,14 @@
   bool vocab_in_s;
   bool sparse_emit;
   bool no_pool;
+  int walk_gather_keys;
   static bool flag(const char *name) {
     const char *e = getenv(name);
     return e && atoi(e) != 0;
   }
   static const EnvOptions &get() {
-    static const EnvOptions o{flag("WP_ARENA_GUARD"), flag("WP_VOCAB_IN_S"), flag("WP_SPARSE_EMIT"), flag("WP_NO_CONTEXT_POOL")};
+    static const EnvOptions o{flag("WP_ARENA_GUARD"), flag("WP_VOCAB_IN_S"), flag("WP_SPARSE_EMIT"), flag("WP_NO_CONTEXT_POOL"),
+                               getenv("WP_WALK_GATHER_KEYS") ? atoi(getenv("WP_WALK_GATHER_KEYS")) & 3 : 0};
     return o;
   }
 };
@@ -132,6 +134,7 @@
 }
 
 constexpr int kScalars = 56;
+constexpr int kMirrorAnchors = kScalars, kMirrorAnchorGap = kScalars + 1, kMirrorWords = kScalars + 2;
 constexpr int kScalarCps = 0;
 constexpr int kScalarAlphabet = 1;
 constexpr int kScalarInvalid = 2;
@@ -209,7 +212,7 @@
 };
 
 enum SideEvent { kEvFork, kEvJoin, kEvScalars, kEvKeysFree, kEvPartition, kEvTrieNodes, kEvLargeSorted, kEvKeysBuilt, kEvCandCount,
-                 kEvSpine, kEvKept, kEvSorted, kEvListBuilt, kEvRoundDone, kSideEvents };
+                 kEvSpine, kEvKept, kEvSorted, kEvListBuilt, kEvRoundDone, kEvAnchorScalars, kSideEvents };
 enum TimingMark { kMarkStart, kMarkCounted, kMarkSymbols, kMarkSorted, kMarkLcp, kMarkScanned, kMarkWalked, kMarkNormStart,
                   kMarkRound0, kTimingMarks, kMarkNormEnd = kMarkStart };
 
@@ -313,6 +316,7 @@
   wp_walk_stats walk;
   wp_refine_stats refine;
   wp_refine_sched sched;
+  wp_walk_keys wkeys;
   wp_inputs_stats inputs;
   int32_t inputs_call;
   wp_mask_stats mask;
@@ -337,6 +341,7 @@
   bool indexed_round0 = false;
   bool sort_blanks = false;
   bool late_refine = WP_LATE_REFINE_DEFAULT != 0;
+  int walk_gather_keys = -1;
   int normalize = 0;
   int n_devices = 1;
   EncodeStats stats{};
@@ -507,7 +512,7 @@
   WP_HIP(hipMalloc(&c->d_code, 512 + 256 + kDecodeTableBytes));
   WP_HIP(hipHostMalloc(&c->h_code, 512 + 256 + kDecodeTableBytes));
   WP_HIP(hipMalloc(&c->d_symhist, sizeof(uint32_t) * 256));
-  WP_HIP(hipHostMalloc(&c->h_scalars, sizeof(uint32_t) * kScalars));
+  WP_HIP(hipHostMalloc(&c->h_scalars, sizeof(uint32_t) * kMirrorWords));
   for (auto &e : c->ev) WP_HIP(hipEventCreate(&e));
   upload_vocab_tables(c.get(), v->hv);
   return c;
@@ -526,6 +531,10 @@
   queue_scalars(c, last, c->stream);
   WP_HIP(hipStreamSynchronize(c->stream));
 }
+static void queue_anchor_scalars(Context *c, hipStream_t st) {
+  static_assert(kScalarAnchorGap == kScalarAnchors + 1 && kMirrorAnchorGap == kMirrorAnchors + 1, "one copy of two words");
+  WP_HIP(hipMemcpyAsync(c->h_scalars + kMirrorAnchors, c->d_scalars + kScalarAnchors, 2 * sizeof(uint32_t), hipMemcpyDeviceToHost, st));
+}
 static void clear_scalars(Context *c, int first, int last, hipStream_t st) {
   WP_HIP(hipMemsetAsync(c->d_scalars + first, 0, sizeof(uint32_t) * (scalar_end(last) - first), st));
 }
diff --git a/wordpiece_amd/csrc/encoder.hip b/wordpiece_amd/csrc/encoder.hip
--- a/wordpiece_amd/csrc/encoder.hip
+++ b/wordpiece_amd/csrc/encoder.hip
@@ -158,6 +158,13 @@
     case WP_OPT_INDEXED_ROUND0: v->indexed_round0 = value != 0; return WP_OK;
     case WP_OPT_SORT_BLANKS: v->sort_blanks = value != 0; return WP_OK;
     case WP_OPT_LATE_REFINE: v->late_refine = value != 0; return WP_OK;
+    case WP_OPT_WALK_GATHER_KEYS:
+      if (value < 0 || value > 3) {
+        g_last_error = "WP_OPT_WALK_GATHER_KEYS: 0 (default), 1 (the walk as it was), 2 or 3 (the anchor key list)";
+        return WP_ERR_ARG;
+      }
+      v->walk_gather_keys = static_cast<int>(value);
+      return WP_OK;
     case WP_OPT_NORMALIZE:
       if (!known_norm_flags(value)) {
         g_last_error = "WP_OPT_NORMALIZE: unknown flag bits (WP_NORM_CLEAN | WP_NORM_LOWER | WP_NORM_STRIP_ACCENTS)";
@@ -223,6 +230,15 @@
     return WP_ERR_ARG;
   }
   *out = v->stats.sched;
+  return WP_OK;
+}
+
+int wp_get_walk_keys(const wp_vocab *v, wp_walk_keys *out) {
+  if (!v || !out) {
+    g_last_error = "wp_get_walk_keys: NULL handle or out pointer";
+    return WP_ERR_ARG;
+  }
+  *out = v->stats.wkeys;
   return WP_OK;
 }
 
@@ -1736,6 +1752,7 @@
       total.refine.n_large_entries = sum.n_large_entries + st.refine.n_large_entries;
     }
     if (i == 0) total.sched = st.sched;
+    if (i == 0) total.wkeys = st.wkeys;
     total.rounds = std::max(total.rounds, st.rounds);
     if (next_up.valid()) {
       const std::string err = next_up.get();
diff --git a/wordpiece_amd/csrc/linear_path.h b/wordpiece_amd/csrc/linear_path.h
--- a/wordpiece_amd/csrc/linear_path.h
+++ b/wordpiece_amd/csrc/linear_path.h
@@ -101,6 +101,8 @@
   bool full, prune, use_trie, key_lookup, keys_only, window_store, use_digit_bytes, staged_possible, sparse_emit;
   bool early_refine;
   bool wide_ran = false;
+  bool key_list = false, late_rank = false, side_scalars = false, anchor_scalars_queued = false;
+  int walk_opt = 0;
   uint32_t need_depth;
   int M, P, P_cap, bucket_shift, bucket_shift_all, key_shift, key_shift_all, hb_n, win_mid;
   unsigned sl_tiles, sl_groups, nbuckets, nbuckets_all, nkbuckets, nkbuckets_all;
@@ -117,6 +119,7 @@
   uint32_t *d_sa = nullptr, *d_gdepth = nullptr;
   RankEntry *d_hd_n = nullptr;
   int32_t *d_emit = nullptr, *d_dbg_best = nullptr;
+  uint32_t *d_akey = nullptr;
   uint32_t *d_anchors = nullptr, *d_anchor_cnt = nullptr, *d_anchor_tmp = nullptr, *d_emit_cnt = nullptr, *d_emit_tmp = nullptr,
            *d_blk_cnt = nullptr, *d_blk_off = nullptr, *d_tile_scratch = nullptr;
   uint32_t *AS0 = nullptr, *AS1 = nullptr, *AG = nullptr, *AD0 = nullptr, *AD1 = nullptr, *LA = nullptr, *LB = nullptr, *d_tdep = nullptr;
@@ -181,6 +184,10 @@
     key_lookup = use_trie && !v->keep_debug && kKeyBits <= 32;
     keys_only = key_lookup && !v->indexed_round0 && sizeof(SymT) == 1;
     early_refine = keys_only && !v->late_refine;
+    walk_opt = v->walk_gather_keys >= 0 ? v->walk_gather_keys : EnvOptions::get().walk_gather_keys;
+    key_list = key_lookup && n > kRadixSmallN && (walk_opt == 2 || walk_opt == 3);
+    late_rank = key_lookup && (walk_opt == 0 || walk_opt == 3);
+    side_scalars = walk_opt != 1;
     sl_tiles = cdiv(n, kSlTile);
     sl_groups = cdiv(sl_tiles, kSlGroup);
     P = kStepsPerMark * M + 1;
@@ -369,10 +376,19 @@
     hipLaunchKernelGGL(anchor_count_kernel, dim3(atiles), dim3(kBlock), 0, as, d_cls, static_cast<const uint8_t *>(nullptr),
                        n_text, d_anchor_cnt);
     device_exclusive_scan(d_anchor_cnt, d_anchor_cnt, atiles, d_anchor_tmp, c->d_scalars + kScalarAnchors, as);
+    if (key_list) {
+      d_akey = VB;
+      if (as == st && (keys_only || vals == VB)) WP_HIP(hipStreamWaitEvent(st, c->evs[kEvKeysFree], 0));
+    }
     hipLaunchKernelGGL(anchor_write_kernel, dim3(atiles), dim3(kBlock), 0, as, d_cls, static_cast<const uint8_t *>(nullptr),
-                       n_text, d_anchor_cnt, d_anchors);
+                       n_text, d_anchor_cnt, d_anchors, reinterpret_cast<const uint32_t *>(KA), d_akey);
     hipLaunchKernelGGL(anchor_gap_kernel, dim3(std::min<size_t>(atiles, 1024)), dim3(kBlock), 0, as, d_anchors,
                        c->d_scalars + kScalarAnchors, n_text, d_cls, hv.soft.empty() ? 1 : 0, c->d_scalars + kScalarAnchorGap);
+    if (side_scalars) {
+      queue_anchor_scalars(c, as);
+      WP_HIP(hipEventRecord(c->evs[kEvAnchorScalars], as));
+      anchor_scalars_queued = true;
+    }
   }
 
   void symbols_and_keys() {
@@ -1108,7 +1124,8 @@
                        d_wp_tiles, d_ns_tiles, d_gap_a, d_gap_b, d_anchor_cnt);
     hipLaunchKernelGGL(suffix_min_kernel, dim3(2), dim3(1024), 0, st, d_wp_tiles, d_ns_tiles, static_cast<size_t>(rtiles));
     device_exclusive_scan(d_anchor_cnt, d_anchor_cnt, atiles, d_anchor_tmp, c->d_scalars + kScalarAnchors, st);
-    hipLaunchKernelGGL(anchor_write_kernel, dim3(atiles), dim3(kBlock), 0, st, d_cls, d_aflags, n_text, d_anchor_cnt, d_anchors);
+    hipLaunchKernelGGL(anchor_write_kernel, dim3(atiles), dim3(kBlock), 0, st, d_cls, d_aflags, n_text, d_anchor_cnt, d_anchors,
+                       reinterpret_cast<const uint32_t *>(KA), d_akey);
     WP_LAUNCH_CHECK();
     fetch_scalars(c, kScalarAnchors);
     wa.aflags = d_aflags;
@@ -1116,6 +1133,28 @@
     wa.ns_from_tile = d_ns_tiles;
     S.anchor_mode = 1;
     return c->h_scalars[kScalarAnchors];
+  }
+
+  template <bool WIDE, bool OFFS>
+  void launch_lean_keys(const WalkArgs &wa, unsigned sblocks, size_t acap, int32_t *d_ctmp, const uint32_t *d_wide_cnt) {
+    uint2 *spill = OFFS ? d_ospill : nullptr, *cspan = OFFS ? d_cspan : nullptr;
+    if (wa.akey) {
+      hipLaunchKernelGGL(HIP_KERNEL_NAME(walk_lean_kernel<WIDE, OFFS, true>), dim3(sblocks), dim3(kBlock), 0, st, wa, d_anchors,
+                         c->d_scalars + kScalarAnchors, acap, d_ctmp, d_blk_cnt, d_wide_cnt, spill, cspan);
+    } else {
+      hipLaunchKernelGGL(HIP_KERNEL_NAME(walk_lean_kernel<WIDE, OFFS, false>), dim3(sblocks), dim3(kBlock), 0, st, wa, d_anchors,
+                         c->d_scalars + kScalarAnchors, acap, d_ctmp, d_blk_cnt, d_wide_cnt, spill, cspan);
+    }
+  }
+  void launch_lean(const WalkArgs &wa, unsigned sblocks, size_t acap, int32_t *d_ctmp, const uint32_t *d_wide_cnt) {
+    const bool offs = offs_unit >= 0;
+    if (d_wide_cnt) {
+      if (offs) launch_lean_keys<true, true>(wa, sblocks, acap, d_ctmp, d_wide_cnt);
+      else launch_lean_keys<true, false>(wa, sblocks, acap, d_ctmp, d_wide_cnt);
+    } else {
+      if (offs) launch_lean_keys<false, true>(wa, sblocks, acap, d_ctmp, nullptr);
+      else launch_lean_keys<false, false>(wa, sblocks, acap, d_ctmp, nullptr);
+    }
   }
 
   int32_t *walk(size_t *n_ids_out) {
@@ -1127,9 +1166,16 @@
                 key_lookup ? reinterpret_cast<const uint32_t *>(KA) : nullptr, ksteps, drop_blanks ? 1 : 0};
     S.anchor_mode = 0;
     join();
-    fetch_scalars(c, kScalarAnchorGap);
-    size_t n_anchors = c->h_scalars[kScalarAnchors];
-    const size_t max_anchor_gap = c->h_scalars[kScalarAnchorGap];
+    size_t n_anchors, max_anchor_gap;
+    if (anchor_scalars_queued) {
+      WP_HIP(hipEventSynchronize(c->evs[kEvAnchorScalars]));
+      n_anchors = c->h_scalars[kMirrorAnchors];
+      max_anchor_gap = c->h_scalars[kMirrorAnchorGap];
+    } else {
+      fetch_scalars(c, kScalarAnchorGap);
+      n_anchors = c->h_scalars[kScalarAnchors];
+      max_anchor_gap = c->h_scalars[kScalarAnchorGap];
+    }
     S.walk.max_anchor_gap = static_cast<int32_t>(max_anchor_gap);
     const bool all_hard = hv.soft.empty();
     bool staged = staged_possible && max_anchor_gap <= kMaxAnchorGap;
@@ -1143,6 +1189,17 @@
     S.n_anchors = static_cast<int64_t>(n_anchors);
     const size_t acap = std::max<size_t>(n_anchors, 1);
     const bool offs = offs_unit >= 0;
+    wa.akey = staged ? d_akey : nullptr;
+    wa.late_rank = late_rank ? 1 : 0;
+    S.wkeys.from_list = wa.akey ? 1 : 0;
+    S.wkeys.reason = wa.akey ? WP_WALK_KEYS_LIST
+                     : walk_opt < 2 ? WP_WALK_KEYS_OPTION
+                     : !key_lookup ? WP_WALK_KEYS_LAYOUT
+                     : !d_akey ? WP_WALK_KEYS_SMALL_TEXT
+                               : WP_WALK_KEYS_SPARSE_WALK;
+    S.wkeys.late_rank = (staged && late_rank) ? 1 : 0;
+    S.wkeys.side_scalars = anchor_scalars_queued ? 1 : 0;
+    S.wkeys.capacity = d_akey ? static_cast<int64_t>(n + 16) : 0;
     if (staged) {
       int32_t *d_ctmp = reinterpret_cast<int32_t *>(X0);
       const unsigned sblocks = cdiv(acap, static_cast<size_t>(kWbWords));
@@ -1159,22 +1216,13 @@
         if (offs) {
           hipLaunchKernelGGL(HIP_KERNEL_NAME(walk_wide_kernel<true>), wgrid, dim3(kBlock), 0, st, wa_all, d_anchors, c->d_scalars + kScalarAnchors,
                              d_wide_list, c->d_scalars + kScalarWideWords, d_wide_cnt, d_ospill);
-          hipLaunchKernelGGL(HIP_KERNEL_NAME(walk_lean_kernel<true, true>), dim3(sblocks), dim3(kBlock), 0, st, wa, d_anchors,
-                             c->d_scalars + kScalarAnchors, acap, d_ctmp, d_blk_cnt, d_wide_cnt, d_ospill, d_cspan);
         } else {
           hipLaunchKernelGGL(HIP_KERNEL_NAME(walk_wide_kernel<false>), wgrid, dim3(kBlock), 0, st, wa_all, d_anchors, c->d_scalars + kScalarAnchors,
                              d_wide_list, c->d_scalars + kScalarWideWords, d_wide_cnt, static_cast<uint2 *>(nullptr));
-          hipLaunchKernelGGL(HIP_KERNEL_NAME(walk_lean_kernel<true, false>), dim3(sblocks), dim3(kBlock), 0, st, wa, d_anchors,
-                             c->d_scalars + kScalarAnchors, acap, d_ctmp, d_blk_cnt, d_wide_cnt, static_cast<uint2 *>(nullptr),
-                             static_cast<uint2 *>(nullptr));
         }
-      } else if (offs) {
-        hipLaunchKernelGGL(HIP_KERNEL_NAME(walk_lean_kernel<false, true>), dim3(sblocks), dim3(kBlock), 0, st, wa, d_anchors,
-                           c->d_scalars + kScalarAnchors, acap, d_ctmp, d_blk_cnt, static_cast<const uint32_t *>(nullptr), d_ospill, d_cspan);
+        launch_lean(wa, sblocks, acap, d_ctmp, d_wide_cnt);
       } else {
-        hipLaunchKernelGGL(HIP_KERNEL_NAME(walk_lean_kernel<false, false>), dim3(sblocks), dim3(kBlock), 0, st, wa, d_anchors,
-                           c->d_scalars + kScalarAnchors, acap, d_ctmp, d_blk_cnt, static_cast<const uint32_t *>(nullptr),
-                           static_cast<uint2 *>(nullptr), static_cast<uint2 *>(nullptr));
+        launch_lean(wa, sblocks, acap, d_ctmp, nullptr);
       }
       device_exclusive_scan(d_blk_cnt, d_blk_off, sblocks, d_emit_tmp, c->d_scalars + kScalarIds, st);
       if (offs) {
diff --git a/wordpiece_amd/csrc/scanline.h b/wordpiece_amd/csrc/scanline.h
--- a/wordpiece_amd/csrc/scanline.h
+++ b/wordpiece_amd/csrc/scanline.h
@@ -441,8 +441,8 @@
   return lo - 1;
 }
 
-__device__ __forceinline__ int32_t step_raw(const StepTable &st, uint32_t r, bool prefix) {
-  const int2 e = st.bfast[r >> st.shift];
+__device__ __forceinline__ int2 step_entry(const StepTable &st, uint32_t r) { return st.bfast[r >> st.shift]; }
+__device__ __forceinline__ int32_t step_raw_of(const StepTable &st, const int2 e, uint32_t r, bool prefix) {
   if (e.x >= kStepNeeded) return prefix ? e.x : e.y;
   const int n = e.x & 0x7fffffff;
   int lo = e.y, hi = e.y + n;
@@ -451,6 +451,9 @@
     if (st.pstart[md] <= r) lo = md + 1; else hi = md;
   }
   return prefix ? st.pval_prefix[lo - 1] : st.pval_suffix[lo - 1];
+}
+__device__ __forceinline__ int32_t step_raw(const StepTable &st, uint32_t r, bool prefix) {
+  return step_raw_of(st, step_entry(st, r), r, prefix);
 }
 
 
diff --git a/wordpiece_amd/csrc/walk.h b/wordpiece_amd/csrc/walk.h
--- a/wordpiece_amd/csrc/walk.h
+++ b/wordpiece_amd/csrc/walk.h
@@ -27,6 +27,8 @@
   const uint32_t *pkey;
   StepTable ksteps;
   int blanks_dropped;
+  const uint32_t *akey;
+  int late_rank;
 };
 
 __device__ __forceinline__ void check_blank_lookup(const WalkArgs &a, uint8_t cls) {
@@ -320,10 +322,22 @@
 
 __global__ __launch_bounds__(kBlock) void anchor_write_kernel(uint8_t *__restrict__ cls, const uint8_t *__restrict__ aflags,
                                                               size_t n, const uint32_t *__restrict__ tile_prefix,
-                                                              uint32_t *__restrict__ anchors) {
+                                                              uint32_t *__restrict__ anchors, const uint32_t *__restrict__ pkey,
+                                                              uint32_t *__restrict__ akey) {
   __shared__ uint32_t sm[8];
   const size_t i = static_cast<size_t>(blockIdx.x) * kAnchorTile + static_cast<size_t>(threadIdx.x) * kAnchorBytes;
   uint32_t m = anchor_mask16(cls, aflags, n, i);
+  uint32_t keys[kAnchorBytes] = {};
+  if (akey && m) {
+#pragma unroll
+    for (int q = 0; q < kAnchorBytes / 4; q++) {
+      const uint4 v = *reinterpret_cast<const uint4 *>(pkey + i + 4 * q);
+      keys[4 * q] = v.x;
+      keys[4 * q + 1] = v.y;
+      keys[4 * q + 2] = v.z;
+      keys[4 * q + 3] = v.w;
+    }
+  }
   if (i < n) {
     uint32_t w[4] = {0, 0, 0, 0};
     const int cnt = static_cast<int>(min(static_cast<size_t>(kAnchorBytes), n - i));
@@ -355,6 +369,17 @@
   }
   uint32_t tot;
   uint32_t o = tile_prefix[blockIdx.x] + block_excl_sum(static_cast<uint32_t>(__popc(m)), sm, tot);
+  if (akey) {
+#pragma unroll
+    for (int j = 0; j < kAnchorBytes; j++) {
+      if ((m >> j) & 1u) {
+        anchors[o] = static_cast<uint32_t>(i + j);
+        akey[o] = keys[j];
+        o++;
+      }
+    }
+    return;
+  }
   while (m) {
     const int j = __ffs(static_cast<int>(m)) - 1;
     m &= m - 1;
@@ -1000,7 +1025,7 @@
   assemble_word_lists<kWbWords, WIDE>(a.emit, anchors, a0, na, stage, cnt, sm, ctmp, blk_cnt, woff, wstart);
 }
 
-template <bool WIDE, bool OFFS = false>
+template <bool WIDE, bool OFFS = false, bool KEYS = false>
 __global__ __launch_bounds__(kBlock) void walk_lean_kernel(WalkArgs a, const uint32_t *__restrict__ anchors,
                                                            const uint32_t *__restrict__ n_anchors_dev, size_t cap,
                                                            int32_t *__restrict__ ctmp, uint32_t *__restrict__ blk_cnt,
@@ -1023,12 +1048,15 @@
                        : 0;
   const bool stop_at_blank = !a.aflags && a.all_hard;
   int widx = wbase + lane;
+  const bool late_rank = a.pkey && a.late_rank;
   uint32_t p = 0, since = 0;
+  uint32_t key = 0;
   Out o{stage + widx, a.emit, 0, 0, kWbWords};
   auto take = [&](int wd) {
     widx = wd;
     const size_t k = a0 + static_cast<size_t>(wd);
     const uint32_t start = anchors[k];
+    if (KEYS) key = a.akey[k];
     p = since = start;
     o = Out{stage + wd, a.emit + start, 0, 0, kWbWords};
     if constexpr (OFFS) o.spans = spans + start;
@@ -1048,11 +1076,21 @@
     if (active) {
       bool done = true;
       if (p < end) {
-        const uint32_t key = step_key(a, p);
-        const uint32_t r = rank_of(a.rank[p]);
+        if (!KEYS) key = step_key(a, p);
+        int2 ke = int2{0, 0};
+        if (KEYS) ke = step_entry(a.ksteps, key);
+        uint32_t r = 0;
+        if (!late_rank) r = rank_of(a.rank[p]);
         uint32_t cw[4];
         __builtin_memcpy(cw, a.cls + p, 16);
-        const int32_t raw = step_value_of(a, key, r, (cw[0] & kClsWordPrefix) != 0);
+        if (!KEYS && a.pkey) ke = step_entry(a.ksteps, key);
+        const bool prefix = (cw[0] & kClsWordPrefix) != 0;
+        int32_t raw = kStepNeeded;
+        if (a.pkey) raw = step_raw_of(a.ksteps, ke, key, prefix);
+        if (raw == kStepNeeded) {
+          if (late_rank) r = rank_of(a.rank[p]);
+          raw = step_raw(a.steps, r, prefix);
+        }
         check_blank_lookup(a, static_cast<uint8_t>(cw[0]));
         const int32_t id = step_id(a.steps, raw);
         bool fast = id >= 0 && wp_in_bounds(id < a.n_tokens, kSiteTokenId);
@@ -1102,6 +1140,7 @@
           p = static_cast<uint32_t>(s.p);
           since = static_cast<uint32_t>(s.since);
         }
+        if (KEYS && !done) key = a.pkey[p];
       }
       if (done) {
         cnt[widx] = o.c;
```
